# knagrecha/saturn

Hardware: AMD Instinct MI355X
Metric: samples_per_s (higher is better)
Workload: dtype bf16; 1 GPU; model=gptj-6b, global_batch=16, seq_len=512, parallelism=dp1, optimizer=fused_sgd

## Files before the change

saturn_amd/models/gptj.py:

```python

from __future__ import annotations


import os
from dataclasses import dataclass

import torch
import torch.nn as nn

from saturn_amd.ops.functional import (
    fused_gelu,
    FusedLayerNorm,
    apply_rope,
    causal_attention,
    fused_add3,
    fused_cross_entropy,
    rope_tables,
    FusedDropout,
    FusedEmbedding,
    gptj_mlp,
    mlp_fused_supported,
    gptj_branches,
    gptj_branches_supported,
)


@dataclass
class GPTJConfig:
    vocab_size: int = 50400
    n_ctx: int = 512
    n_embd: int = 4096
    n_head: int = 16
    n_layer: int = 28
    rotary_dim: int = 64
    embd_pdrop: float = 0.0
    resid_pdrop: float = 0.0


class GPTJAttention(nn.Module):
    def __init__(self, cfg: GPTJConfig):
        super().__init__()
        self.n_head = cfg.n_head
        self.head_dim = cfg.n_embd // cfg.n_head
        self.rotary_dim = cfg.rotary_dim
        E = cfg.n_embd
        self.q_proj = nn.Linear(E, E, bias=False)
        self.k_proj = nn.Linear(E, E, bias=False)
        self.v_proj = nn.Linear(E, E, bias=False)
        self.out_proj = nn.Linear(E, E, bias=False)
        self.n_ctx = cfg.n_ctx
        self._rope_f32 = rope_tables(cfg.n_ctx, cfg.rotary_dim)

    def _rope(self, device):
        if self._rope_f32[0].device != device:
            self._rope_f32 = tuple(t.to(device) for t in self._rope_f32)
        return self._rope_f32

    def forward(self, x):
        B, T, E = x.shape
        H, D = self.n_head, self.head_dim
        q = self.q_proj(x).view(B, T, H, D)
        k = self.k_proj(x).view(B, T, H, D)
        v = self.v_proj(x).view(B, T, H, D)
        cos, sin = self._rope(x.device)
        q = apply_rope(q, cos, sin)
        k = apply_rope(k, cos, sin)
        q = q.transpose(1, 2)
        k = k.transpose(1, 2)
        v = v.transpose(1, 2)
        o = causal_attention(q, k, v)
        o = o.transpose(1, 2).reshape(B, T, -1)
        return self.out_proj(o)


class GPTJMLP(nn.Module):
    def __init__(self, cfg: GPTJConfig):
        super().__init__()
        E = cfg.n_embd
        self.fc_in = nn.Linear(E, 4 * E)
        self.fc_out = nn.Linear(4 * E, E)

    @staticmethod
    def _plain_linear(m) -> bool:
        return type(m) is nn.Linear and not (
            m._forward_hooks
            or m._forward_pre_hooks
            or m._backward_hooks
            or m._backward_pre_hooks
        )

    def _use_fused(self, x) -> bool:
        if os.environ.get("SAMD_MLP_FUSED", "1") == "0":
            return False
        fi, fo = self.fc_in, self.fc_out
        return (
            x.is_cuda
            and self._plain_linear(fi)
            and self._plain_linear(fo)
            and mlp_fused_supported(x, fi.weight, fi.bias, fo.weight, fo.bias)
        )

    def forward(self, x):
        if self._use_fused(x):
            fi, fo = self.fc_in, self.fc_out
            return gptj_mlp(x, fi.weight, fi.bias, fo.weight, fo.bias)
        return self.fc_out(fused_gelu(self.fc_in(x)))


class GPTJBlock(nn.Module):

    def __init__(self, cfg: GPTJConfig):
        super().__init__()
        self.ln_1 = FusedLayerNorm(cfg.n_embd)
        self.attn = GPTJAttention(cfg)
        self.mlp = GPTJMLP(cfg)
        self.drop = FusedDropout(cfg.resid_pdrop)

    @staticmethod
    def _hooked(m) -> bool:
        return bool(
            m._forward_hooks
            or m._forward_pre_hooks
            or m._backward_hooks
            or m._backward_pre_hooks
        )

    def _use_fused(self, h) -> bool:
        if (os.environ.get("SAMD_MLP_FUSED", "1") == "0"
                or os.environ.get("SAMD_BLOCK_FUSED", "1") == "0"):
            return False
        attn, mlp = self.attn, self.mlp
        if type(attn) is not GPTJAttention or type(mlp) is not GPTJMLP:
            return False
        if not (h.is_cuda and h.dtype == torch.bfloat16 and h.dim() == 3):
            return False
        if self.drop.p != 0.0:
            return False
        from saturn_amd.parallel.sequence import sp_world

        if sp_world() != 1:
            return False
        if any(self._hooked(m) for b in (attn, mlp, self.drop) for m in b.modules()):
            return False
        projs = (attn.q_proj, attn.k_proj, attn.v_proj, attn.out_proj)
        fi, fo = mlp.fc_in, mlp.fc_out
        if not all(GPTJMLP._plain_linear(m) for m in (*projs, fi, fo)):
            return False
        E = h.shape[-1]
        if any(m.bias is not None or m.weight.shape != (E, E)
               or m.weight.dtype != torch.bfloat16 or not m.weight.is_cuda
               for m in projs):
            return False
        return mlp_fused_supported(
            h, fi.weight, fi.bias, fo.weight, fo.bias
        ) and gptj_branches_supported(
            h, attn.n_head, attn.rotary_dim, attn._rope_f32[0].shape[0]
        )

    def forward(self, x):
        h = self.ln_1(x)
        if self._use_fused(h):
            attn, mlp = self.attn, self.mlp
            cos, sin = attn._rope(h.device)
            a, m = gptj_branches(
                h, attn.q_proj.weight, attn.k_proj.weight, attn.v_proj.weight,
                attn.out_proj.weight, mlp.fc_in.weight, mlp.fc_in.bias,
                mlp.fc_out.weight, mlp.fc_out.bias, cos, sin, attn.n_head,
            )
            return fused_add3(x, a, m)
        return fused_add3(x, self.drop(self.attn(h)), self.drop(self.mlp(h)))


class GPTJForCausalLM(nn.Module):
    def __init__(self, cfg: GPTJConfig):
        super().__init__()
        self.cfg = cfg
        self.wte = FusedEmbedding(cfg.vocab_size, cfg.n_embd)
        self.drop = FusedDropout(cfg.embd_pdrop)
        self.h = nn.ModuleList(GPTJBlock(cfg) for _ in range(cfg.n_layer))
        self.ln_f = FusedLayerNorm(cfg.n_embd)
        self.lm_head = nn.Linear(cfg.n_embd, cfg.vocab_size, bias=True)
        self.apply(self._init)

    @staticmethod
    def _init(m):
        if isinstance(m, nn.Linear):
            nn.init.normal_(m.weight, std=0.02)
            if m.bias is not None:
                nn.init.zeros_(m.bias)
        elif isinstance(m, nn.Embedding):
            nn.init.normal_(m.weight, std=0.02)

    def forward(self, input_ids):
        x = self.drop(self.wte(input_ids))
        for block in self.h:
            x = block(x)
        x = self.ln_f(x)
        return self.lm_head(x)


def pretraining_loss(logits, labels):
    return fused_cross_entropy(logits, labels, shift=True)


class _EmbedStage(nn.Module):
    def __init__(self, wte):
        super().__init__()
        self.wte = wte

    def forward(self, input_ids):
        return self.wte(input_ids)


class _HeadStage(nn.Module):
    def __init__(self, ln_f, lm_head):
        super().__init__()
        self.ln_f = ln_f
        self.lm_head = lm_head

    def forward(self, x):
        return self.lm_head(self.ln_f(x))


def as_sequential(model: GPTJForCausalLM) -> nn.Sequential:
    return nn.Sequential(
        _EmbedStage(model.wte), *model.h, _HeadStage(model.ln_f, model.lm_head)
    )


def get_gptj_model(kwargs=None):
    kwargs = kwargs or {}
    cfg = GPTJConfig(
        n_layer=kwargs.get("n_layer", 28),
        n_embd=kwargs.get("n_embd", 4096),
        n_head=kwargs.get("n_head", 16),
        n_ctx=kwargs.get("n_ctx", 512),
        vocab_size=kwargs.get("vocab_size", 50400),
        rotary_dim=kwargs.get("rotary_dim", 64),
        embd_pdrop=kwargs.get("embd_pdrop", 0.0),
        resid_pdrop=kwargs.get("resid_pdrop", 0.0),
    )
    torch.manual_seed(kwargs.get("seed", 0))
    return GPTJForCausalLM(cfg)


class SyntheticTokens(torch.utils.data.Dataset):

    def __init__(self, n: int, seq_len: int, vocab: int, seed: int = 1):
        g = torch.Generator().manual_seed(seed)
        self.data = torch.randint(0, vocab, (n, seq_len), generator=g)

    def __len__(self):
        return len(self.data)

    def __getitem__(self, i):
        return self.data[i]


def _collate(batch):
    x = torch.stack(batch)
    return x, x.clone()


def make_token_dataloader(batch_size=8, seq_len=512, vocab=50400, n_batches=64):
    def get_dataloader():
        return torch.utils.data.DataLoader(
            SyntheticTokens(batch_size * n_batches, seq_len, vocab),
            batch_size=batch_size,
            shuffle=False,
            collate_fn=_collate,
        )

    return get_dataloader
```

saturn_amd/ops/csrc/attention.hip:

```cpp

#include <torch/extension.h>
#include <ATen/hip/HIPContext.h>

#include "common.h"

namespace samd {

typedef __attribute__((ext_vector_type(8))) short bf16x8;
typedef __attribute__((ext_vector_type(4))) float f32x4;

constexpr int QBLK = 64;
constexpr int KBLK = 32;
constexpr int WROWS = 16;

struct TStr {
  long sb, sh, st;
};
static TStr str_of(const at::Tensor& t) {
  return TStr{t.stride(0), t.stride(1), t.stride(2)};
}


typedef __attribute__((ext_vector_type(4))) short bf16x4;

__device__ __forceinline__ unsigned lds_addr32(const unsigned short* p) {
  return (unsigned)(unsigned long long)(
      __attribute__((address_space(3))) const unsigned short*)p;
}

template <int P1, int P2>
__device__ __forceinline__ void tr16_bfrag2(const unsigned short* t1_row0,
                                            const unsigned short* t2_row0,
                                            int lane, bf16x8& o1, bf16x8& o2) {
  const int src_row = (lane >> 2) & 3;
  const int src_col = 4 * (lane & 3);
  const unsigned a0 = lds_addr32(t1_row0 + src_row * P1 + src_col);
  const unsigned a1 = a0 + 4u * P1 * 2u;
  const unsigned b0 = lds_addr32(t2_row0 + src_row * P2 + src_col);
  const unsigned b1 = b0 + 4u * P2 * 2u;
  bf16x4 v0, v1, w0, w1;
  asm volatile(
      "ds_read_b64_tr_b16 %0, %4\n\t"
      "ds_read_b64_tr_b16 %1, %5\n\t"
      "ds_read_b64_tr_b16 %2, %6\n\t"
      "ds_read_b64_tr_b16 %3, %7\n\t"
      "s_waitcnt lgkmcnt(0)"
      : "=&v"(v0), "=&v"(v1), "=&v"(w0), "=&v"(w1)
      : "v"(a0), "v"(a1), "v"(b0), "v"(b1)
      : "memory");
  o1 = __builtin_shufflevector(v0, v1, 0, 1, 2, 3, 4, 5, 6, 7);
  o2 = __builtin_shufflevector(w0, w1, 0, 1, 2, 3, 4, 5, 6, 7);
}

template <int ROWPITCH>
__device__ __forceinline__ bf16x8 tr16_bfrag(const unsigned short* tile_row0,
                                             int lane) {
  const int src_row = (lane >> 2) & 3;
  const int src_col = 4 * (lane & 3);
  const unsigned a0 =
      lds_addr32(tile_row0 + src_row * ROWPITCH + src_col);
  const unsigned a1 = a0 + 4u * ROWPITCH * 2u;
  bf16x4 v0, v1;
  asm volatile(
      "ds_read_b64_tr_b16 %0, %2\n\t"
      "ds_read_b64_tr_b16 %1, %3\n\t"
      "s_waitcnt lgkmcnt(0)"
      : "=&v"(v0), "=&v"(v1)
      : "v"(a0), "v"(a1)
      : "memory");
  return __builtin_shufflevector(v0, v1, 0, 1, 2, 3, 4, 5, 6, 7);
}

template <int D>
struct AttnLds {
  unsigned short k[KBLK][D + 8];
  unsigned short v[KBLK][D + 8];
  unsigned short p[4][WROWS][KBLK];
};

template <int D>
__launch_bounds__(256, 2)
__global__ void attn_fwd_kernel(const unsigned short* __restrict__ Q,
                                const unsigned short* __restrict__ K,
                                const unsigned short* __restrict__ V,
                                unsigned short* __restrict__ O,
                                float* __restrict__ LSE, int T, int n_heads,
                                int n_kv, float scale, int causal,
                                int kv_len, TStr qs, TStr ks, TStr vs,
                                TStr os) {
  extern __shared__ __attribute__((aligned(16))) char smem[];
  AttnLds<D>& lds = *reinterpret_cast<AttnLds<D>*>(smem);

  const int lane = threadIdx.x & 63;
  const int wid = threadIdx.x >> 6;
  const int q0_block = blockIdx.y * QBLK;
  const int q0 = q0_block + wid * WROWS;
  const long bh = blockIdx.x;
  const long b = bh / n_heads, h = bh % n_heads;
  const long h_kv = h * n_kv / n_heads;
  const unsigned short* Qh = Q + b * qs.sb + h * qs.sh;
  const unsigned short* Kh = K + b * ks.sb + h_kv * ks.sh;
  const unsigned short* Vh = V + b * vs.sb + h_kv * vs.sh;

  const int r = lane & 15;
  const int qg = lane >> 4;

  bf16x8 frag_q[D / 32];
#pragma unroll
  for (int ds = 0; ds < D / 32; ++ds) {
    const unsigned short* src = Qh + (long)(q0 + r) * qs.st + ds * 32 + qg * 8;
    frag_q[ds] = *reinterpret_cast<const bf16x8*>(src);
  }

  f32x4 otile[D / 16];
#pragma unroll
  for (int dt = 0; dt < D / 16; ++dt) otile[dt] = {0.f, 0.f, 0.f, 0.f};

  float m_reg[4] = {-INFINITY, -INFINITY, -INFINITY, -INFINITY};
  float l_reg[4] = {0.f, 0.f, 0.f, 0.f};

  const int kv_end = causal ? (q0_block + QBLK) : T;
  constexpr int CHUNKS = (KBLK * D) / (256 * 8);
  bf16x8 stg_k[CHUNKS], stg_v[CHUNKS];
#pragma unroll
  for (int c = 0; c < CHUNKS; ++c) {
    const int idx = (c * 256 + threadIdx.x) * 8;
    const int row = idx / D, col = idx % D;
    stg_k[c] = *reinterpret_cast<const bf16x8*>(Kh + (long)row * ks.st + col);
    stg_v[c] = *reinterpret_cast<const bf16x8*>(Vh + (long)row * vs.st + col);
  }
  for (int kv0 = 0; kv0 < kv_end; kv0 += KBLK) {
    __syncthreads();
#pragma unroll
    for (int c = 0; c < CHUNKS; ++c) {
      const int idx = (c * 256 + threadIdx.x) * 8;
      const int row = idx / D, col = idx % D;
      *reinterpret_cast<bf16x8*>(&lds.k[row][col]) = stg_k[c];
      *reinterpret_cast<bf16x8*>(&lds.v[row][col]) = stg_v[c];
    }
    if (kv0 + KBLK < kv_end) {
#pragma unroll
      for (int c = 0; c < CHUNKS; ++c) {
        const int idx = (c * 256 + threadIdx.x) * 8;
        const int row = idx / D, col = idx % D;
        stg_k[c] = *reinterpret_cast<const bf16x8*>(
            Kh + (long)(kv0 + KBLK + row) * ks.st + col);
        stg_v[c] = *reinterpret_cast<const bf16x8*>(
            Vh + (long)(kv0 + KBLK + row) * vs.st + col);
      }
    }
    __syncthreads();

    f32x4 acc0 = {0.f, 0.f, 0.f, 0.f};
    f32x4 acc1 = {0.f, 0.f, 0.f, 0.f};
#pragma unroll
    for (int ds = 0; ds < D / 32; ++ds) {
      bf16x8 bk0 = *reinterpret_cast<const bf16x8*>(&lds.k[r][ds * 32 + qg * 8]);
      bf16x8 bk1 =
          *reinterpret_cast<const bf16x8*>(&lds.k[16 + r][ds * 32 + qg * 8]);
      acc0 = __builtin_amdgcn_mfma_f32_16x16x32_bf16(frag_q[ds], bk0, acc0, 0, 0, 0);
      acc1 = __builtin_amdgcn_mfma_f32_16x16x32_bf16(frag_q[ds], bk1, acc1, 0, 0, 0);
    }
#pragma unroll
    for (int reg = 0; reg < 4; ++reg) {
      const int row = qg * 4 + reg;
      const int qrow = q0 + row;
      float s0 = acc0[reg] * scale;
      float s1 = acc1[reg] * scale;
      if (causal) {
        if (kv0 + r > qrow) s0 = -INFINITY;
        if (kv0 + 16 + r > qrow) s1 = -INFINITY;
      }
      if (kv0 + r >= kv_len) s0 = -INFINITY;
      if (kv0 + 16 + r >= kv_len) s1 = -INFINITY;
      float tm = fmaxf(s0, s1);
#pragma unroll
      for (int off = 1; off < 16; off <<= 1)
        tm = fmaxf(tm, __shfl_xor(tm, off, 64));
      const float m_new = fmaxf(m_reg[reg], tm);
      const float al =
          (m_reg[reg] == -INFINITY) ? 0.f : __expf(m_reg[reg] - m_new);
      const float p0 = (s0 == -INFINITY) ? 0.f : __expf(s0 - m_new);
      const float p1 = (s1 == -INFINITY) ? 0.f : __expf(s1 - m_new);
      float ps = p0 + p1;
#pragma unroll
      for (int off = 1; off < 16; off <<= 1)
        ps += __shfl_xor(ps, off, 64);
      l_reg[reg] = l_reg[reg] * al + ps;
      m_reg[reg] = m_new;
      lds.p[wid][row][r] = f2us(p0);
      lds.p[wid][row][16 + r] = f2us(p1);
#pragma unroll
      for (int dt = 0; dt < D / 16; ++dt) otile[dt][reg] *= al;
    }

    bf16x8 frag_p = *reinterpret_cast<const bf16x8*>(&lds.p[wid][r][qg * 8]);
#pragma unroll
    for (int dt = 0; dt < D / 16; ++dt) {
      bf16x8 bv = tr16_bfrag<D + 8>(&lds.v[qg * 8][dt * 16], lane);
      otile[dt] = __builtin_amdgcn_mfma_f32_16x16x32_bf16(frag_p, bv, otile[dt], 0, 0, 0);
    }
  }

  unsigned short* Oh = O + b * os.sb + h * os.sh;
#pragma unroll
  for (int reg = 0; reg < 4; ++reg) {
    int row = qg * 4 + reg;
    float linv = 1.f / l_reg[reg];
#pragma unroll
    for (int dt = 0; dt < D / 16; ++dt)
      Oh[(long)(q0 + row) * os.st + dt * 16 + r] =
          f2us(otile[dt][reg] * linv);
  }
  if (r == 0 && LSE != nullptr) {
#pragma unroll
    for (int reg = 0; reg < 4; ++reg)
      LSE[bh * (long)T + q0 + qg * 4 + reg] =
          m_reg[reg] + __logf(l_reg[reg]);
  }
}



typedef __attribute__((ext_vector_type(16))) float f32x16;

template <int D>
struct AttnV2Lds {
  unsigned short k[KBLK][D + 8];
  unsigned short v[KBLK][D + 8];
};

template <int D>
__launch_bounds__(256, 2)
__global__ void attn_fwd_v2_kernel(const unsigned short* __restrict__ Q,
                                   const unsigned short* __restrict__ K,
                                   const unsigned short* __restrict__ V,
                                   unsigned short* __restrict__ O,
                                   float* __restrict__ LSE, int T,
                                   int n_heads, int n_kv, float scale,
                                   int causal, int kv_len, TStr qs,
                                   TStr ks, TStr vs,
                                   TStr os) {
  extern __shared__ __attribute__((aligned(16))) char smem[];
  AttnV2Lds<D>& lds = *reinterpret_cast<AttnV2Lds<D>*>(smem);

  const int lane = threadIdx.x & 63;
  const int wid = threadIdx.x >> 6;
  const int qr = lane & 31;
  const int hi = lane >> 5;
  const long bh = blockIdx.x;
  const long b = bh / n_heads, h = bh % n_heads;
  const long h_kv = h * n_kv / n_heads;
  const int q0_block = blockIdx.y * (4 * 32);
  const int q0 = q0_block + wid * 32;
  const unsigned short* Qh = Q + b * qs.sb + h * qs.sh;
  const unsigned short* Kh = K + b * ks.sb + h_kv * ks.sh;
  const unsigned short* Vh = V + b * vs.sb + h_kv * vs.sh;

  constexpr bool QREG = (D < 256);
  bf16x8 frag_q[QREG ? D / 16 : 1];
  if constexpr (QREG) {
#pragma unroll
    for (int ds = 0; ds < D / 16; ++ds)
      frag_q[ds] = *reinterpret_cast<const bf16x8*>(
          Qh + (long)(q0 + qr) * qs.st + ds * 16 + hi * 8);
  }

  f32x16 oacc[D / 32];
#pragma unroll
  for (int dv = 0; dv < D / 32; ++dv)
#pragma unroll
    for (int e = 0; e < 16; ++e) oacc[dv][e] = 0.f;

  float m_row = -INFINITY, l_row = 0.f;

  constexpr int CHUNKS = (KBLK * D) / (256 * 8);
  bf16x8 stg_k[CHUNKS], stg_v[CHUNKS];
#pragma unroll
  for (int c = 0; c < CHUNKS; ++c) {
    const int idx = (c * 256 + threadIdx.x) * 8;
    const int row = idx / D, col = idx % D;
    stg_k[c] = *reinterpret_cast<const bf16x8*>(Kh + (long)row * ks.st + col);
    stg_v[c] = *reinterpret_cast<const bf16x8*>(Vh + (long)row * vs.st + col);
  }

  const int kv_end = causal ? (q0_block + 4 * 32) : T;
  for (int kv0 = 0; kv0 < kv_end; kv0 += KBLK) {
    __syncthreads();
#pragma unroll
    for (int c = 0; c < CHUNKS; ++c) {
      const int idx = (c * 256 + threadIdx.x) * 8;
      const int row = idx / D, col = idx % D;
      *reinterpret_cast<bf16x8*>(&lds.k[row][col]) = stg_k[c];
      *reinterpret_cast<bf16x8*>(&lds.v[row][col]) = stg_v[c];
    }
    if (kv0 + KBLK < kv_end) {
#pragma unroll
      for (int c = 0; c < CHUNKS; ++c) {
        const int idx = (c * 256 + threadIdx.x) * 8;
        const int row = idx / D, col = idx % D;
        stg_k[c] = *reinterpret_cast<const bf16x8*>(
            Kh + (long)(kv0 + KBLK + row) * ks.st + col);
        stg_v[c] = *reinterpret_cast<const bf16x8*>(
            Vh + (long)(kv0 + KBLK + row) * vs.st + col);
      }
    }
    __syncthreads();

    f32x16 st;
#pragma unroll
    for (int e = 0; e < 16; ++e) st[e] = 0.f;
#pragma unroll
    for (int ds = 0; ds < D / 16; ++ds) {
      bf16x8 ak = *reinterpret_cast<const bf16x8*>(
          &lds.k[qr][ds * 16 + hi * 8]);
      bf16x8 fq;
      if constexpr (QREG)
        fq = frag_q[ds];
      else
        fq = *reinterpret_cast<const bf16x8*>(
            Qh + (long)(q0 + qr) * qs.st + ds * 16 + hi * 8);
      st = __builtin_amdgcn_mfma_f32_32x32x16_bf16(ak, fq, st, 0, 0, 0);
    }

    const int q_glob = q0 + qr;
    float p[16];
    float tile_max = -INFINITY;
#pragma unroll
    for (int reg = 0; reg < 16; ++reg) {
      const int key_loc = (reg & 3) + 8 * (reg >> 2) + 4 * hi;
      float sv = st[reg] * scale;
      if ((causal && kv0 + key_loc > q_glob) || kv0 + key_loc >= kv_len)
        sv = -INFINITY;
      p[reg] = sv;
      tile_max = fmaxf(tile_max, sv);
    }
    tile_max = fmaxf(tile_max, __shfl_xor(tile_max, 32, 64));
    const float m_new = fmaxf(m_row, tile_max);
    const float alpha = (m_row == -INFINITY) ? 0.f : __expf(m_row - m_new);
    float psum = 0.f;
#pragma unroll
    for (int reg = 0; reg < 16; ++reg) {
      const float pv = (p[reg] == -INFINITY) ? 0.f : __expf(p[reg] - m_new);
      p[reg] = pv;
      psum += pv;
    }
    psum += __shfl_xor(psum, 32, 64);
    l_row = l_row * alpha + psum;
    m_row = m_new;

    unsigned pk[8];
#pragma unroll
    for (int i = 0; i < 8; ++i) {
      const unsigned lo = f2us(p[2 * i]);
      const unsigned hi2 = f2us(p[2 * i + 1]);
      pk[i] = lo | (hi2 << 16);
    }
    bf16x8 pa[2];
#pragma unroll
    for (int g = 0; g < 2; ++g) {
      auto r0 = __builtin_amdgcn_permlane32_swap(pk[4 * g + 0], pk[4 * g + 2],
                                                 false, false);
      auto r1 = __builtin_amdgcn_permlane32_swap(pk[4 * g + 1], pk[4 * g + 3],
                                                 false, false);
      unsigned w0 = r0[0], w1 = r1[0], w2 = r0[1], w3 = r1[1];
      pa[g][0] = (short)(w0 & 0xffff);
      pa[g][1] = (short)(w0 >> 16);
      pa[g][2] = (short)(w1 & 0xffff);
      pa[g][3] = (short)(w1 >> 16);
      pa[g][4] = (short)(w2 & 0xffff);
      pa[g][5] = (short)(w2 >> 16);
      pa[g][6] = (short)(w3 & 0xffff);
      pa[g][7] = (short)(w3 >> 16);
    }

#pragma unroll
    for (int reg = 0; reg < 16; ++reg) {
      const int row = (reg & 3) + 8 * (reg >> 2) + 4 * hi;
      const float al = __shfl(alpha, row, 64);
#pragma unroll
      for (int dv = 0; dv < D / 32; ++dv) oacc[dv][reg] *= al;
    }

#pragma unroll
    for (int dv = 0; dv < D / 32; ++dv) {
#pragma unroll
      for (int g = 0; g < 2; ++g) {
        const int src_row = g * 16 + ((lane >> 4) & 2) * 4 + ((lane >> 2) & 3);
        const int src_col = dv * 32 + ((lane >> 4) & 1) * 16 + 4 * (lane & 3);
        const unsigned a0 = lds_addr32(&lds.v[src_row][src_col]);
        const unsigned a1 = a0 + 4u * (D + 8) * 2u;
        bf16x4 v0, v1;
        asm volatile(
            "ds_read_b64_tr_b16 %0, %2\n\t"
            "ds_read_b64_tr_b16 %1, %3\n\t"
            "s_waitcnt lgkmcnt(0)"
            : "=&v"(v0), "=&v"(v1)
            : "v"(a0), "v"(a1)
            : "memory");
        bf16x8 bv = __builtin_shufflevector(v0, v1, 0, 1, 2, 3, 4, 5, 6, 7);
        oacc[dv] = __builtin_amdgcn_mfma_f32_32x32x16_bf16(pa[g], bv,
                                                           oacc[dv], 0, 0, 0);
      }
    }
  }

  unsigned short* Oh = O + b * os.sb + h * os.sh;
  const float linv_own = 1.f / l_row;
#pragma unroll
  for (int reg = 0; reg < 16; ++reg) {
    const int row = (reg & 3) + 8 * (reg >> 2) + 4 * hi;
    const float linv = __shfl(linv_own, row, 64);
#pragma unroll
    for (int dv = 0; dv < D / 32; ++dv)
      Oh[(long)(q0 + row) * os.st + dv * 32 + qr] = f2us(oacc[dv][reg] * linv);
  }
  if (hi == 0 && LSE != nullptr)
    LSE[bh * (long)T + q0 + qr] = m_row + __logf(l_row);
}



static bool env_is(const char* name, char c) {
  const char* e = getenv(name);
  return e && e[0] == c;
}
static bool sw_v2() {
  static const bool v = !env_is("SAMD_ATTN_V2", '0');
  return v;
}
static bool sw_tr16() {
  static const bool v = !env_is("SAMD_ATTN_BWD_TR16", '0');
  return v;
}
static bool sw_dq_gkv() {
  static const bool v = env_is("SAMD_ATTN_DQ_GKV", '1');
  return v;
}
static bool sw_vl2() {
  static const bool v = env_is("SAMD_ATTN_BWD_VL2", '1');
  return v;
}
static bool fwd_is_v2(int T, int D) {
  return sw_v2() && T % 128 == 0 && D <= 128;
}
static bool bwd_is_tr16(int D) { return sw_tr16() && D <= 128; }
static bool bwd_is_vl2(int D) { return sw_vl2() && D <= 128; }
static bool dq_is_gkv(int D) { return sw_dq_gkv() && D > 128; }

std::string attn_dispatch(int64_t T, int64_t D) {
  TORCH_CHECK(T > 0 && T % QBLK == 0, "attn_dispatch: T must be a multiple of 64");
  TORCH_CHECK(D == 64 || D == 128 || D == 256, "attn_dispatch: D in {64,128,256}");
  const int t = (int)T, d = (int)D;
  const std::string ds = std::to_string(d);
  const bool gkv = dq_is_gkv(d);
  return std::string(fwd_is_v2(t, d) ? "attn_fwd_v2_kernel<" : "attn_fwd_kernel<") +
         ds + "> attn_delta_kernel<" + ds + "> attn_bwd_kernel<" + ds + "," +
         (bwd_is_tr16(d) ? "1," : "0,") + (bwd_is_vl2(d) ? "1>" : "0>") +
         " attn_dq_kernel<" + ds + "," +
         (!gkv && bwd_is_tr16(d) ? "1," : "0,") + (gkv ? "1>" : "0>");
}

std::vector<at::Tensor> attn_fwd(at::Tensor q, at::Tensor k, at::Tensor v,
                                 bool causal, int64_t kv_len) {
  TORCH_CHECK(q.is_cuda() && q.scalar_type() == at::kBFloat16,
              "attn_fwd: bf16 only");
  TORCH_CHECK(q.dim() == 4, "attn_fwd: [B, H, T, D]");
  TORCH_CHECK(q.stride(3) == 1 && k.stride(3) == 1 && v.stride(3) == 1,
              "attn_fwd: innermost dim must be dense");
  const int B = (int)q.size(0), H = (int)q.size(1), T = (int)q.size(2),
            D = (int)q.size(3);
  const int Hkv = (int)k.size(1);
  TORCH_CHECK(H % Hkv == 0, "attn_fwd: q heads must be a multiple of kv heads");
  TORCH_CHECK(k.size(2) == T, "attn_fwd: q/k length mismatch");
  TORCH_CHECK(T % QBLK == 0, "attn_fwd: T must be a multiple of 64");
  if (kv_len <= 0) kv_len = T;
  TORCH_CHECK(kv_len <= T, "attn_fwd: kv_len exceeds padded T");
  TORCH_CHECK(D == 64 || D == 128 || D == 256, "attn_fwd: D in {64,128,256}");
  TORCH_CHECK((reinterpret_cast<uintptr_t>(q.data_ptr()) & 15) == 0 &&
              q.stride(2) % 8 == 0 && k.stride(2) % 8 == 0 &&
              v.stride(2) % 8 == 0, "attn_fwd: rows must be 16-B aligned");

  auto o_phys = at::empty({B, T, H, D}, q.options());
  auto o = o_phys.permute({0, 2, 1, 3});
  auto lse = at::empty({B, H, T}, q.options().dtype(at::kFloat));
  auto stream = at::hip::getCurrentHIPStream();
  const float scale = 1.f / sqrtf((float)D);

  if (fwd_is_v2(T, D)) {
    dim3 grid2(B * H, T / 128), block2(256);
#define LAUNCH_V2(DD)                                                        \
    do {                                                                     \
      size_t shmem = sizeof(AttnV2Lds<DD>);                                  \
      hipLaunchKernelGGL((attn_fwd_v2_kernel<DD>), grid2, block2, shmem,     \
                         stream.stream(),                                    \
                         reinterpret_cast<const unsigned short*>(q.data_ptr()), \
                         reinterpret_cast<const unsigned short*>(k.data_ptr()), \
                         reinterpret_cast<const unsigned short*>(v.data_ptr()), \
                         reinterpret_cast<unsigned short*>(o.data_ptr()),    \
                         lse.data_ptr<float>(), T, H, Hkv, scale,            \
                         causal ? 1 : 0, (int)kv_len, str_of(q), str_of(k),  \
                         str_of(v), str_of(o));                              \
    } while (0)
    if (D == 64) LAUNCH_V2(64);
    else LAUNCH_V2(128);
#undef LAUNCH_V2
    return {o, lse};
  }
  dim3 grid(B * H, T / QBLK), block(256);

#define LAUNCH(DD)                                                          \
  do {                                                                      \
    size_t shmem = sizeof(AttnLds<DD>);                                     \
    hipLaunchKernelGGL((attn_fwd_kernel<DD>), grid, block, shmem,           \
                       stream.stream(),                                     \
                       reinterpret_cast<const unsigned short*>(q.data_ptr()), \
                       reinterpret_cast<const unsigned short*>(k.data_ptr()), \
                       reinterpret_cast<const unsigned short*>(v.data_ptr()), \
                       reinterpret_cast<unsigned short*>(o.data_ptr()),     \
                       lse.data_ptr<float>(), T, H, Hkv, scale,             \
                       causal ? 1 : 0, (int)kv_len, str_of(q), str_of(k),   \
                       str_of(v), str_of(o));                               \
  } while (0)

  if (D == 64) LAUNCH(64);
  else if (D == 128) LAUNCH(128);
  else LAUNCH(256);
#undef LAUNCH
  return {o, lse};
}

}


namespace samd {

namespace bwd {
constexpr int KB = 64;
constexpr int QT = 32;
}

template <int D, bool HASV>
struct AttnBwdLds {
  unsigned short kt[bwd::KB][D + 8];
  unsigned short vt[HASV ? bwd::KB : 1][D + 8];
  unsigned short qt[bwd::QT][D + 8];
  unsigned short dot[bwd::QT][D + 8];
  unsigned short pt[4][16][bwd::QT + 8];
  unsigned short dst[bwd::KB][bwd::QT + 8];
  float lse_t[bwd::QT];
  float delta_t[bwd::QT];
};


template <int D>
__global__ void attn_delta_kernel(const unsigned short* __restrict__ dO,
                                  const unsigned short* __restrict__ O,
                                  float* __restrict__ delta, int T,
                                  int n_heads, TStr dos, TStr os) {
  const int lane = threadIdx.x & 63;
  const int wid = threadIdx.x >> 6;
  const long bh = blockIdx.y;
  const long b = bh / n_heads, h = bh % n_heads;
  const unsigned short* dOh = dO + b * dos.sb + h * dos.sh;
  const unsigned short* Oh = O + b * os.sb + h * os.sh;
  constexpr int EPL = D / 64;
  for (int t = blockIdx.x * 4 + wid; t < T; t += gridDim.x * 4) {
    float acc = 0.f;
    if constexpr (EPL >= 4) {
#pragma unroll
      for (int c = 0; c < EPL / 4; ++c) {
        const int off = (lane * (EPL / 4) + c * 64) * 4;
        bf16x4 a = *reinterpret_cast<const bf16x4*>(dOh + (long)t * dos.st + off);
        bf16x4 o4 = *reinterpret_cast<const bf16x4*>(Oh + (long)t * os.st + off);
#pragma unroll
        for (int e = 0; e < 4; ++e)
          acc += us2f((unsigned short)a[e]) * us2f((unsigned short)o4[e]);
      }
    } else {
#pragma unroll
      for (int e = 0; e < EPL; ++e) {
        const int off = lane * EPL + e;
        acc += us2f(dOh[(long)t * dos.st + off]) *
               us2f(Oh[(long)t * os.st + off]);
      }
    }
    acc = wave_allsum(acc);
    if (lane == 0) delta[bh * (long)T + t] = acc;
  }
}

template <int D, bool TR16, bool VL2>
__launch_bounds__(256, 2)
__global__ void attn_bwd_kernel(const unsigned short* __restrict__ dO,
                                const unsigned short* __restrict__ Q,
                                const unsigned short* __restrict__ K,
                                const unsigned short* __restrict__ V,
                                const float* __restrict__ LSE,
                                const float* __restrict__ DELTA,
                                unsigned short* __restrict__ dK,
                                unsigned short* __restrict__ dV,
                                float* __restrict__ dKf,
                                float* __restrict__ dVf, int T, int n_heads,
                                int n_kv, float scale, int causal,
                                int kv_len, TStr dos,
                                TStr qs, TStr ks, TStr vs,
                                TStr dks, TStr dvs) {
  using namespace bwd;
  extern __shared__ __attribute__((aligned(16))) char smem[];
  constexpr bool HASV = (D <= 128) && !VL2;
  AttnBwdLds<D, HASV>& lds = *reinterpret_cast<AttnBwdLds<D, HASV>*>(smem);

  const int lane = threadIdx.x & 63;
  const int wid = threadIdx.x >> 6;
  const int r = lane & 15;
  const int qg = lane >> 4;
  const int kv0 = blockIdx.y * KB;
  const long bh = blockIdx.x;
  const long b = bh / n_heads, h = bh % n_heads;
  const long h_kv = h * n_kv / n_heads;
  const unsigned short* Qh = Q + b * qs.sb + h * qs.sh;
  const unsigned short* Kh = K + b * ks.sb + h_kv * ks.sh;
  const unsigned short* Vh = V + b * vs.sb + h_kv * vs.sh;
  const unsigned short* dOh = dO + b * dos.sb + h * dos.sh;
  const float* lse_h = LSE + bh * (long)T;
  const float* del_h = DELTA + bh * (long)T;

  {
    constexpr int CHUNKS = (KB * D) / (256 * 8);
#pragma unroll
    for (int c = 0; c < CHUNKS; ++c) {
      int idx = (c * 256 + threadIdx.x) * 8;
      int row = idx / D, col = idx % D;
      *reinterpret_cast<bf16x8*>(&lds.kt[row][col]) =
          *reinterpret_cast<const bf16x8*>(
              Kh + (long)(kv0 + row) * ks.st + col);
      if constexpr (HASV)
        *reinterpret_cast<bf16x8*>(&lds.vt[row][col]) =
            *reinterpret_cast<const bf16x8*>(
                Vh + (long)(kv0 + row) * vs.st + col);
    }
  }

  f32x4 acc_dv[D / 16], acc_dk[D / 16];
#pragma unroll
  for (int dt = 0; dt < D / 16; ++dt) {
    acc_dv[dt] = {0.f, 0.f, 0.f, 0.f};
    acc_dk[dt] = {0.f, 0.f, 0.f, 0.f};
  }

  const int q_start = causal ? kv0 : 0;
  for (int q0 = q_start; q0 < T; q0 += QT) {
    __syncthreads();
    {
      constexpr int CHUNKS = (QT * D) / (256 * 8);
#pragma unroll
      for (int c = 0; c < CHUNKS; ++c) {
        int idx = (c * 256 + threadIdx.x) * 8;
        int row = idx / D, col = idx % D;
        *reinterpret_cast<bf16x8*>(&lds.qt[row][col]) =
            *reinterpret_cast<const bf16x8*>(
                Qh + (long)(q0 + row) * qs.st + col);
        *reinterpret_cast<bf16x8*>(&lds.dot[row][col]) =
            *reinterpret_cast<const bf16x8*>(
                dOh + (long)(q0 + row) * dos.st + col);
      }
      if (threadIdx.x < QT) {
        lds.lse_t[threadIdx.x] = lse_h[q0 + threadIdx.x];
        lds.delta_t[threadIdx.x] = del_h[q0 + threadIdx.x];
      }
    }
    __syncthreads();

#pragma unroll
    for (int n = 0; n < 2; ++n) {
      f32x4 st = {0.f, 0.f, 0.f, 0.f};
      f32x4 dpt = {0.f, 0.f, 0.f, 0.f};
#pragma unroll
      for (int ds = 0; ds < D / 32; ++ds) {
        bf16x8 ak = *reinterpret_cast<const bf16x8*>(
            &lds.kt[wid * 16 + r][ds * 32 + qg * 8]);
        bf16x8 av;
        if constexpr (HASV)
          av = *reinterpret_cast<const bf16x8*>(
              &lds.vt[wid * 16 + r][ds * 32 + qg * 8]);
        else
          av = *reinterpret_cast<const bf16x8*>(
              Vh + (long)(kv0 + wid * 16 + r) * vs.st + ds * 32 + qg * 8);
        bf16x8 bq = *reinterpret_cast<const bf16x8*>(
            &lds.qt[n * 16 + r][ds * 32 + qg * 8]);
        bf16x8 bdo = *reinterpret_cast<const bf16x8*>(
            &lds.dot[n * 16 + r][ds * 32 + qg * 8]);
        st = __builtin_amdgcn_mfma_f32_16x16x32_bf16(ak, bq, st, 0, 0, 0);
        dpt = __builtin_amdgcn_mfma_f32_16x16x32_bf16(av, bdo, dpt, 0, 0, 0);
      }
#pragma unroll
      for (int reg = 0; reg < 4; ++reg) {
        const int key_loc = qg * 4 + reg;
        const int key_glob = kv0 + wid * 16 + key_loc;
        const int q_glob = q0 + n * 16 + r;
        float p = 0.f;
        if ((!causal || q_glob >= key_glob) && key_glob < kv_len) {
          p = __expf(scale * st[reg] - lds.lse_t[n * 16 + r]);
        }
        const float dsv = p * (dpt[reg] - lds.delta_t[n * 16 + r]) * scale;
        lds.pt[wid][key_loc][n * 16 + r] = f2us(p);
        lds.dst[wid * 16 + key_loc][n * 16 + r] = f2us(dsv);
      }
    }

    {
      bf16x8 ap = *reinterpret_cast<const bf16x8*>(&lds.pt[wid][r][qg * 8]);
      bf16x8 adst =
          *reinterpret_cast<const bf16x8*>(&lds.dst[wid * 16 + r][qg * 8]);
#pragma unroll
      for (int dt = 0; dt < D / 16; ++dt) {
        bf16x8 bdo, bq;
        if constexpr (TR16) {
          tr16_bfrag2<D + 8, D + 8>(&lds.dot[qg * 8][dt * 16],
                                    &lds.qt[qg * 8][dt * 16], lane, bdo, bq);
        } else {
#pragma unroll
          for (int j = 0; j < 8; ++j) {
            bdo[j] = (short)lds.dot[qg * 8 + j][dt * 16 + r];
            bq[j] = (short)lds.qt[qg * 8 + j][dt * 16 + r];
          }
        }
        acc_dv[dt] =
            __builtin_amdgcn_mfma_f32_16x16x32_bf16(ap, bdo, acc_dv[dt], 0, 0, 0);
        acc_dk[dt] =
            __builtin_amdgcn_mfma_f32_16x16x32_bf16(adst, bq, acc_dk[dt], 0, 0, 0);
      }
    }

    __syncthreads();
  }

  if (n_kv != n_heads) {
    float* dKh = dKf + b * dks.sb + h_kv * dks.sh;
    float* dVh = dVf + b * dvs.sb + h_kv * dvs.sh;
#pragma unroll
    for (int reg = 0; reg < 4; ++reg) {
      const int key_glob = kv0 + wid * 16 + qg * 4 + reg;
#pragma unroll
      for (int dt = 0; dt < D / 16; ++dt) {
        atomicAdd(&dKh[(long)key_glob * dks.st + dt * 16 + r],
                  acc_dk[dt][reg]);
        atomicAdd(&dVh[(long)key_glob * dvs.st + dt * 16 + r],
                  acc_dv[dt][reg]);
      }
    }
  } else {
    unsigned short* dKh = dK + b * dks.sb + h * dks.sh;
    unsigned short* dVh = dV + b * dvs.sb + h * dvs.sh;
#pragma unroll
    for (int reg = 0; reg < 4; ++reg) {
      const int key_glob = kv0 + wid * 16 + qg * 4 + reg;
#pragma unroll
      for (int dt = 0; dt < D / 16; ++dt) {
        dKh[(long)key_glob * dks.st + dt * 16 + r] = f2us(acc_dk[dt][reg]);
        dVh[(long)key_glob * dvs.st + dt * 16 + r] = f2us(acc_dv[dt][reg]);
      }
    }
  }
}

namespace dq {
constexpr int QB = 64;
constexpr int KT = 32;
}

template <int D, bool GKV>
struct AttnDqLds {
  unsigned short qt[GKV ? 1 : dq::QB][D + 8];
  unsigned short dot[GKV ? 1 : dq::QB][D + 8];
  unsigned short kt[dq::KT][D + 8];
  unsigned short vt[GKV ? 1 : dq::KT][D + 8];
  float lse_t[dq::QB];
  float delta_t[dq::QB];
};

template <int D, bool TR16, bool GKV>
__launch_bounds__(256, GKV ? 3 : (D <= 128 ? 2 : 1))
__global__ void attn_dq_kernel(const unsigned short* __restrict__ dO,
                               const unsigned short* __restrict__ Q,
                               const unsigned short* __restrict__ K,
                               const unsigned short* __restrict__ V,
                               const float* __restrict__ LSE,
                               const float* __restrict__ DELTA,
                               unsigned short* __restrict__ dQ16, int T,
                               int n_heads, int n_kv, float scale, int causal,
                               int kv_len, TStr dos, TStr qs, TStr ks,
                               TStr vs, TStr dqs) {
  using namespace dq;
  extern __shared__ __attribute__((aligned(16))) char smem[];
  AttnDqLds<D, GKV>& lds = *reinterpret_cast<AttnDqLds<D, GKV>*>(smem);

  const int lane = threadIdx.x & 63;
  const int wid = threadIdx.x >> 6;
  const int r = lane & 15;
  const int qg = lane >> 4;
  const int q0 = blockIdx.y * QB;
  const long bh = blockIdx.x;
  const long b = bh / n_heads, h = bh % n_heads;
  const long h_kv = h * n_kv / n_heads;
  const unsigned short* Qh = Q + b * qs.sb + h * qs.sh;
  const unsigned short* Kh = K + b * ks.sb + h_kv * ks.sh;
  const unsigned short* Vh = V + b * vs.sb + h_kv * vs.sh;
  const unsigned short* dOh = dO + b * dos.sb + h * dos.sh;
  const float* lse_h = LSE + bh * (long)T;
  const float* del_h = DELTA + bh * (long)T;

  {
    if constexpr (!GKV) {
      constexpr int CHUNKS = (QB * D) / (256 * 8);
#pragma unroll
      for (int c = 0; c < CHUNKS; ++c) {
        int idx = (c * 256 + threadIdx.x) * 8;
        int row = idx / D, col = idx % D;
        *reinterpret_cast<bf16x8*>(&lds.qt[row][col]) =
            *reinterpret_cast<const bf16x8*>(Qh + (long)(q0 + row) * qs.st + col);
        *reinterpret_cast<bf16x8*>(&lds.dot[row][col]) =
            *reinterpret_cast<const bf16x8*>(
                dOh + (long)(q0 + row) * dos.st + col);
      }
    }
    if (threadIdx.x < QB) {
      lds.lse_t[threadIdx.x] = lse_h[q0 + threadIdx.x];
      lds.delta_t[threadIdx.x] = del_h[q0 + threadIdx.x];
    }
  }

  f32x4 acc[D / 16];
#pragma unroll
  for (int dt = 0; dt < D / 16; ++dt) acc[dt] = {0.f, 0.f, 0.f, 0.f};

  const int k_end = causal ? (q0 + QB < T ? q0 + QB : T) : T;
  for (int k0 = 0; k0 < k_end; k0 += KT) {
    __syncthreads();
    {
      constexpr int CHUNKS = (KT * D) / (256 * 8);
#pragma unroll
      for (int c = 0; c < CHUNKS; ++c) {
        int idx = (c * 256 + threadIdx.x) * 8;
        int row = idx / D, col = idx % D;
        *reinterpret_cast<bf16x8*>(&lds.kt[row][col]) =
            *reinterpret_cast<const bf16x8*>(
                Kh + (long)(k0 + row) * ks.st + col);
        if constexpr (!GKV)
          *reinterpret_cast<bf16x8*>(&lds.vt[row][col]) =
              *reinterpret_cast<const bf16x8*>(
                  Vh + (long)(k0 + row) * vs.st + col);
      }
    }
    __syncthreads();

    if (causal && k0 > q0 + wid * 16 + 15) continue;

    float ds_sub[2][4];
#pragma unroll
    for (int n = 0; n < 2; ++n) {
      f32x4 st = {0.f, 0.f, 0.f, 0.f};
      f32x4 dpt = {0.f, 0.f, 0.f, 0.f};
#pragma unroll
      for (int ds_ = 0; ds_ < D / 32; ++ds_) {
        bf16x8 ak = *reinterpret_cast<const bf16x8*>(
            &lds.kt[n * 16 + r][ds_ * 32 + qg * 8]);
        bf16x8 av, bq, bdo;
        if constexpr (GKV) {
          av = *reinterpret_cast<const bf16x8*>(
              Vh + (long)(k0 + n * 16 + r) * vs.st + ds_ * 32 + qg * 8);
          bq = *reinterpret_cast<const bf16x8*>(
              Qh + (long)(q0 + wid * 16 + r) * qs.st + ds_ * 32 + qg * 8);
          bdo = *reinterpret_cast<const bf16x8*>(
              dOh + (long)(q0 + wid * 16 + r) * dos.st + ds_ * 32 + qg * 8);
        } else {
          av = *reinterpret_cast<const bf16x8*>(
              &lds.vt[n * 16 + r][ds_ * 32 + qg * 8]);
          bq = *reinterpret_cast<const bf16x8*>(
              &lds.qt[wid * 16 + r][ds_ * 32 + qg * 8]);
          bdo = *reinterpret_cast<const bf16x8*>(
              &lds.dot[wid * 16 + r][ds_ * 32 + qg * 8]);
        }
        st = __builtin_amdgcn_mfma_f32_16x16x32_bf16(ak, bq, st, 0, 0, 0);
        dpt = __builtin_amdgcn_mfma_f32_16x16x32_bf16(av, bdo, dpt, 0, 0, 0);
      }
      const int q_glob = q0 + wid * 16 + r;
      const float l_q = lds.lse_t[wid * 16 + r];
      const float d_q = lds.delta_t[wid * 16 + r];
#pragma unroll
      for (int reg = 0; reg < 4; ++reg) {
        const int key_glob = k0 + n * 16 + qg * 4 + reg;
        float p = 0.f;
        if ((!causal || q_glob >= key_glob) && key_glob < kv_len)
          p = __expf(scale * st[reg] - l_q);
        ds_sub[n][reg] = p * (dpt[reg] - d_q) * scale;
      }
    }

    unsigned pk[2][2];
#pragma unroll
    for (int n = 0; n < 2; ++n) {
      pk[n][0] = (unsigned)f2us(ds_sub[n][0]) |
                 ((unsigned)f2us(ds_sub[n][1]) << 16);
      pk[n][1] = (unsigned)f2us(ds_sub[n][2]) |
                 ((unsigned)f2us(ds_sub[n][3]) << 16);
    }
    const int a = (qg & 1) * 2;
    const int nsrc = qg >> 1;
    const int s0 = a * 16 + r;
    const int s1 = (a + 1) * 16 + r;
    unsigned rr[4][2];
#pragma unroll
    for (int nn = 0; nn < 2; ++nn) {
      rr[nn * 2 + 0][0] = (unsigned)__shfl((int)pk[nn][0], s0, 64);
      rr[nn * 2 + 0][1] = (unsigned)__shfl((int)pk[nn][1], s0, 64);
      rr[nn * 2 + 1][0] = (unsigned)__shfl((int)pk[nn][0], s1, 64);
      rr[nn * 2 + 1][1] = (unsigned)__shfl((int)pk[nn][1], s1, 64);
    }
    bf16x8 ads;
#pragma unroll
    for (int j = 0; j < 8; ++j) {
      const int src = (j >= 4) ? 1 : 0;
      const int reg = j & 3;
      const unsigned u = rr[nsrc * 2 + src][reg >> 1];
      ads[j] = (short)((reg & 1) ? (u >> 16) : (u & 0xffffu));
    }

#pragma unroll
    for (int dt = 0; dt < D / 16; ++dt) {
      bf16x8 bk;
      if constexpr (TR16) {
        bk = tr16_bfrag<D + 8>(&lds.kt[qg * 8][dt * 16], lane);
      } else {
#pragma unroll
        for (int j = 0; j < 8; ++j)
          bk[j] = (short)lds.kt[qg * 8 + j][dt * 16 + r];
      }
      acc[dt] = __builtin_amdgcn_mfma_f32_16x16x32_bf16(ads, bk, acc[dt], 0, 0, 0);
    }
  }

  unsigned short* dQh = dQ16 + b * dqs.sb + h * dqs.sh;
#pragma unroll
  for (int reg = 0; reg < 4; ++reg) {
    const int q_glob = q0 + wid * 16 + qg * 4 + reg;
#pragma unroll
    for (int dt = 0; dt < D / 16; ++dt)
      dQh[(long)q_glob * dqs.st + dt * 16 + r] = f2us(acc[dt][reg]);
  }
}

std::vector<at::Tensor> attn_bwd(at::Tensor dout, at::Tensor q, at::Tensor k,
                                 at::Tensor v, at::Tensor o, at::Tensor lse,
                                 bool causal, int64_t kv_len) {
  using namespace bwd;
  TORCH_CHECK(q.is_cuda() && q.scalar_type() == at::kBFloat16);
  const int B = (int)q.size(0), H = (int)q.size(1), T = (int)q.size(2),
            D = (int)q.size(3);
  const int Hkv = (int)k.size(1);
  TORCH_CHECK(H % Hkv == 0);
  TORCH_CHECK(T % KB == 0, "attn_bwd: T must be a multiple of 64");
  if (kv_len <= 0) kv_len = T;
  TORCH_CHECK(kv_len <= T, "attn_bwd: kv_len exceeds padded T");
  TORCH_CHECK(D == 64 || D == 128 || D == 256);
  TORCH_CHECK(dout.stride(3) == 1 && q.stride(3) == 1 && k.stride(3) == 1 &&
              v.stride(3) == 1, "attn_bwd: innermost dim must be dense");
  TORCH_CHECK(dout.stride(2) % 8 == 0 && q.stride(2) % 8 == 0 &&
              k.stride(2) % 8 == 0 && v.stride(2) % 8 == 0);

  auto delta = at::empty({B, H, T}, q.options().dtype(at::kFloat));
  auto dq = at::empty({B, T, H, D}, q.options()).permute({0, 2, 1, 3});
  const bool gqa = Hkv != H;
  auto dk = at::empty({B, T, Hkv, D}, k.options()).permute({0, 2, 1, 3});
  auto dv = at::empty({B, T, Hkv, D}, v.options()).permute({0, 2, 1, 3});
  at::Tensor dk_f32, dv_f32;
  if (gqa) {
    dk_f32 = at::zeros({B, T, Hkv, D}, q.options().dtype(at::kFloat))
                 .permute({0, 2, 1, 3});
    dv_f32 = at::zeros({B, T, Hkv, D}, q.options().dtype(at::kFloat))
                 .permute({0, 2, 1, 3});
  }
  auto stream = at::hip::getCurrentHIPStream();
  const float scale = 1.f / sqrtf((float)D);
  dim3 grid(B * H, T / KB), block(256);

#define BWD_ARGS                                                             \
    stream.stream(),                                                         \
    reinterpret_cast<const unsigned short*>(dout.data_ptr()),                \
    reinterpret_cast<const unsigned short*>(q.data_ptr()),                   \
    reinterpret_cast<const unsigned short*>(k.data_ptr()),                   \
    reinterpret_cast<const unsigned short*>(v.data_ptr()),                   \
    lse.data_ptr<float>(), delta.data_ptr<float>(),                          \
    reinterpret_cast<unsigned short*>(dk.data_ptr()),                        \
    reinterpret_cast<unsigned short*>(dv.data_ptr()),                        \
    gqa ? dk_f32.data_ptr<float>() : nullptr,                                \
    gqa ? dv_f32.data_ptr<float>() : nullptr, T, H, Hkv,                     \
    scale, causal ? 1 : 0, (int)kv_len, str_of(dout), str_of(q),             \
    str_of(k), str_of(v),                                                    \
    gqa ? str_of(dk_f32) : str_of(dk),                                       \
    gqa ? str_of(dv_f32) : str_of(dv)

#define LAUNCH_B(DD)                                                         \
  do {                                                                       \
    dim3 dgrid(std::min((T + 3) / 4, 2048), B * H), dblock(256);             \
    hipLaunchKernelGGL((attn_delta_kernel<DD>), dgrid, dblock, 0,            \
                       stream.stream(),                                      \
                       reinterpret_cast<const unsigned short*>(dout.data_ptr()), \
                       reinterpret_cast<const unsigned short*>(o.data_ptr()), \
                       delta.data_ptr<float>(), T, H, str_of(dout),          \
                       str_of(o));                                           \
                                                           \
    const bool gkv = dq_is_gkv(DD);                                          \
    size_t SH_DQ = gkv ? sizeof(AttnDqLds<DD, true>)                         \
                       : sizeof(AttnDqLds<DD, false>);                       \
    static bool dq_attr_##DD = [] {                                          \
      hipFuncSetAttribute(                                                   \
          reinterpret_cast<const void*>(&attn_dq_kernel<DD, false, false>),  \
          hipFuncAttributeMaxDynamicSharedMemorySize,                        \
          (int)sizeof(AttnDqLds<DD, false>));                                \
      hipFuncSetAttribute(                                                   \
          reinterpret_cast<const void*>(&attn_dq_kernel<DD, true, false>),   \
          hipFuncAttributeMaxDynamicSharedMemorySize,                        \
          (int)sizeof(AttnDqLds<DD, false>));                                \
      return true;                                                           \
    }();                                                                     \
    (void)dq_attr_##DD;                                                      \
    {                                                                        \
      dim3 qgrid(B * H, T / dq::QB), qblock(256);                            \
      if (gkv)                                                               \
        hipLaunchKernelGGL((attn_dq_kernel<DD, false, true>), qgrid,         \
                           qblock, SH_DQ, stream.stream(),                   \
                           reinterpret_cast<const unsigned short*>(dout.data_ptr()), \
                           reinterpret_cast<const unsigned short*>(q.data_ptr()), \
                           reinterpret_cast<const unsigned short*>(k.data_ptr()), \
                           reinterpret_cast<const unsigned short*>(v.data_ptr()), \
                           lse.data_ptr<float>(), delta.data_ptr<float>(),   \
                           reinterpret_cast<unsigned short*>(dq.data_ptr()), \
                           T, H, Hkv, scale, causal ? 1 : 0, (int)kv_len,   \
                           str_of(dout), str_of(q), str_of(k), str_of(v),    \
                           str_of(dq));                                      \
      else if (bwd_is_tr16(DD))                                              \
        hipLaunchKernelGGL((attn_dq_kernel<DD, true, false>), qgrid,         \
                           qblock, SH_DQ, stream.stream(),                   \
                           reinterpret_cast<const unsigned short*>(dout.data_ptr()), \
                           reinterpret_cast<const unsigned short*>(q.data_ptr()), \
                           reinterpret_cast<const unsigned short*>(k.data_ptr()), \
                           reinterpret_cast<const unsigned short*>(v.data_ptr()), \
                           lse.data_ptr<float>(), delta.data_ptr<float>(),   \
                           reinterpret_cast<unsigned short*>(dq.data_ptr()), \
                           T, H, Hkv, scale, causal ? 1 : 0, (int)kv_len,   \
                           str_of(dout), str_of(q), str_of(k), str_of(v),    \
                           str_of(dq));                                      \
      else                                                                   \
        hipLaunchKernelGGL((attn_dq_kernel<DD, false, false>), qgrid,        \
                           qblock, SH_DQ, stream.stream(),                   \
                           reinterpret_cast<const unsigned short*>(dout.data_ptr()), \
                           reinterpret_cast<const unsigned short*>(q.data_ptr()), \
                           reinterpret_cast<const unsigned short*>(k.data_ptr()), \
                           reinterpret_cast<const unsigned short*>(v.data_ptr()), \
                           lse.data_ptr<float>(), delta.data_ptr<float>(),   \
                           reinterpret_cast<unsigned short*>(dq.data_ptr()), \
                           T, H, Hkv, scale, causal ? 1 : 0, (int)kv_len,   \
                           str_of(dout), str_of(q), str_of(k), str_of(v),    \
                           str_of(dq));                                      \
    }                                                                        \
    const bool tr = bwd_is_tr16(DD);                                         \
    const bool vl2 = bwd_is_vl2(DD);                                         \
    constexpr size_t SH_V = sizeof(AttnBwdLds<DD, (DD <= 128)>);             \
    constexpr size_t SH_N = sizeof(AttnBwdLds<DD, false>);                   \
    size_t shmem = vl2 ? SH_N : SH_V;                                        \
    static bool attr_set_##DD = [] {                                         \
      hipFuncSetAttribute(                                                   \
          reinterpret_cast<const void*>(&attn_bwd_kernel<DD, false, false>), \
          hipFuncAttributeMaxDynamicSharedMemorySize, (int)SH_V);            \
      hipFuncSetAttribute(                                                   \
          reinterpret_cast<const void*>(&attn_bwd_kernel<DD, true, false>),  \
          hipFuncAttributeMaxDynamicSharedMemorySize, (int)SH_V);            \
      hipFuncSetAttribute(                                                   \
          reinterpret_cast<const void*>(&attn_bwd_kernel<DD, false, true>),  \
          hipFuncAttributeMaxDynamicSharedMemorySize, (int)SH_N);            \
      hipFuncSetAttribute(                                                   \
          reinterpret_cast<const void*>(&attn_bwd_kernel<DD, true, true>),   \
          hipFuncAttributeMaxDynamicSharedMemorySize, (int)SH_N);            \
      return true;                                                           \
    }();                                                                     \
    (void)attr_set_##DD;                                                     \
    if (tr && vl2)                                                           \
      hipLaunchKernelGGL((attn_bwd_kernel<DD, true, true>), grid, block,     \
                         shmem, BWD_ARGS);                                   \
    else if (tr)                                                             \
      hipLaunchKernelGGL((attn_bwd_kernel<DD, true, false>), grid, block,    \
                         shmem, BWD_ARGS);                                   \
    else if (vl2)                                                            \
      hipLaunchKernelGGL((attn_bwd_kernel<DD, false, true>), grid, block,    \
                         shmem, BWD_ARGS);                                   \
    else                                                                     \
      hipLaunchKernelGGL((attn_bwd_kernel<DD, false, false>), grid, block,   \
                         shmem, BWD_ARGS);                                   \
  } while (0)

  if (D == 64) LAUNCH_B(64);
  else if (D == 128) LAUNCH_B(128);
  else LAUNCH_B(256);
#undef LAUNCH_B
  if (gqa) return {dq, dk_f32.to(at::kBFloat16), dv_f32.to(at::kBFloat16)};
  return {dq, dk, dv};
}

}
```

saturn_amd/ops/csrc/bindings.cpp:

```cpp

#include <torch/extension.h>
#include <vector>

namespace samd {
void fused_sgd(std::vector<at::Tensor> params, std::vector<at::Tensor> grads,
               std::vector<at::Tensor> moms, std::vector<at::Tensor> masters,
               double lr, double momentum, double weight_decay);
void fused_adam(std::vector<at::Tensor> params, std::vector<at::Tensor> grads,
                std::vector<at::Tensor> ms, std::vector<at::Tensor> vs,
                std::vector<at::Tensor> masters, double lr, double beta1,
                double beta2, double eps, double weight_decay, double bc1,
                double bc2);
std::vector<at::Tensor> norm_fwd(at::Tensor x, at::Tensor w,
                                 c10::optional<at::Tensor> b, double eps,
                                 bool rms);
std::vector<at::Tensor> norm_bwd(at::Tensor dy, at::Tensor x, at::Tensor w,
                                 at::Tensor mean, at::Tensor rstd, bool rms,
                                 bool needs_db);
std::vector<at::Tensor> ce_fwd(at::Tensor logits, at::Tensor targets,
                               int64_t Tr, int64_t ignore_index);
at::Tensor ce_bwd(at::Tensor logits, at::Tensor targets, at::Tensor lse,
                  at::Tensor dloss, int64_t Tr, int64_t ignore_index);
void rope_apply(at::Tensor y, at::Tensor x, at::Tensor cos_t, at::Tensor sin_t,
                int64_t t_len, int64_t t_off, bool half_style, bool backward);
at::Tensor gelu_fwd(at::Tensor x);
at::Tensor gelu_bwd(at::Tensor dy, at::Tensor x);
std::vector<at::Tensor> attn_fwd(at::Tensor q, at::Tensor k, at::Tensor v,
                                 bool causal, int64_t kv_len);
std::vector<at::Tensor> attn_bwd(at::Tensor dout, at::Tensor q, at::Tensor k,
                                 at::Tensor v, at::Tensor o, at::Tensor lse,
                                 bool causal, int64_t kv_len);
std::string attn_dispatch(int64_t T, int64_t D);
at::Tensor add3(at::Tensor a, at::Tensor b, at::Tensor c);
at::Tensor swiglu_fwd(at::Tensor gate, at::Tensor up);
std::vector<at::Tensor> swiglu_bwd(at::Tensor dout, at::Tensor gate,
                                   at::Tensor up);
at::Tensor embed_fwd(at::Tensor weight, at::Tensor idx);
at::Tensor embed_bwd(at::Tensor dout, at::Tensor idx, long vocab);
at::Tensor dropout_fwd(at::Tensor x, double p, long seed);
at::Tensor dropout_bwd(at::Tensor dout, double p, long seed);
std::vector<at::Tensor> moe_route_fwd(at::Tensor logits, int64_t top_k,
                                      at::ScalarType out_dtype);
at::Tensor moe_route_bwd(at::Tensor logits, at::Tensor ids,
                         at::Tensor dweights);
std::vector<at::Tensor> moe_sort(at::Tensor ids, int64_t n_expert);
at::Tensor moe_permute_fwd(at::Tensor x, at::Tensor order, int64_t top_k);
at::Tensor moe_permute_bwd(at::Tensor dxs, at::Tensor pos);
at::Tensor moe_combine_fwd(at::Tensor y, at::Tensor weights, at::Tensor pos);
std::vector<at::Tensor> moe_combine_bwd(at::Tensor dout, at::Tensor y,
                                        at::Tensor weights, at::Tensor pos);
std::vector<at::Tensor> mlp_act_bwd(at::Tensor d_act, at::Tensor pre,
                                    bool want_dT, bool want_aT);
std::vector<at::Tensor> transpose_colsum(at::Tensor x, bool want_sum);
std::vector<at::Tensor> mlp_bwd(at::Tensor g, at::Tensor h, at::Tensor pre,
                                at::Tensor W_in, at::Tensor W_out,
                                bool use_tn_in, bool use_tn_out);
void transpose_into(at::Tensor x, at::Tensor dst);
at::Tensor rope_bwd_t(at::Tensor dy, at::Tensor cos_t, at::Tensor sin_t,
                      int64_t t_len, int64_t t_off, int64_t dim,
                      at::Tensor dxT);
std::vector<at::Tensor> gptj_branches_bwd(
    at::Tensor g_a, at::Tensor g_m, at::Tensor h, at::Tensor pre, at::Tensor q,
    at::Tensor k, at::Tensor v, at::Tensor o, at::Tensor lse, at::Tensor Wq,
    at::Tensor Wk, at::Tensor Wv, at::Tensor Wo, at::Tensor W_in,
    at::Tensor W_out, at::Tensor cos_t, at::Tensor sin_t, int64_t t_off,
    bool tn_in, bool tn_out, bool tn_qkv, bool tn_o, bool dh_accum);
}

PYBIND11_MODULE(TORCH_EXTENSION_NAME, m) {
  m.doc() = "saturn_amd hand-written CDNA4 (gfx950) kernels";
  m.def("fused_sgd", &samd::fused_sgd, "fused multi-tensor SGD");
  m.def("fused_adam", &samd::fused_adam, "fused multi-tensor AdamW");
  m.def("norm_fwd", &samd::norm_fwd, "LayerNorm/RMSNorm forward");
  m.def("norm_bwd", &samd::norm_bwd, "LayerNorm/RMSNorm backward");
  m.def("ce_fwd", &samd::ce_fwd, "fused cross-entropy forward");
  m.def("ce_bwd", &samd::ce_bwd, "fused cross-entropy backward");
  m.def("rope_apply", &samd::rope_apply,
        "fused rotary embedding (out-of-place, offset table rows)");
  m.def("gelu_fwd", &samd::gelu_fwd, "fused tanh-approx GELU forward");
  m.def("gelu_bwd", &samd::gelu_bwd, "fused tanh-approx GELU backward");
  m.def("attn_fwd", &samd::attn_fwd, "fused flash attention forward",
        py::arg("q"), py::arg("k"), py::arg("v"), py::arg("causal"),
        py::arg("kv_len") = -1);
  m.def("attn_dispatch", &samd::attn_dispatch,
        "kernel instantiations attn_fwd/attn_bwd launch for (padded T, D)",
        py::arg("T"), py::arg("D"));
  m.def("attn_bwd", &samd::attn_bwd, "fused flash attention backward",
        py::arg("dout"), py::arg("q"), py::arg("k"), py::arg("v"),
        py::arg("o"), py::arg("lse"), py::arg("causal"),
        py::arg("kv_len") = -1);
  m.def("add3", &samd::add3, "fused 3-way residual add");
  m.def("swiglu_fwd", &samd::swiglu_fwd, "fused silu(gate)*up");
  m.def("swiglu_bwd", &samd::swiglu_bwd, "fused SwiGLU backward");
  m.def("embed_fwd", &samd::embed_fwd, "token embedding gather");
  m.def("embed_bwd", &samd::embed_bwd, "embedding scatter-add backward");
  m.def("dropout_fwd", &samd::dropout_fwd, "counter-based fused dropout");
  m.def("dropout_bwd", &samd::dropout_bwd, "dropout backward (mask recompute)");
  m.def("moe_route_fwd", &samd::moe_route_fwd,
        "MoE softmax + top-k + renormalise (ties to the lower expert)");
  m.def("moe_route_bwd", &samd::moe_route_bwd, "MoE routing backward");
  m.def("moe_sort", &samd::moe_sort,
        "stable counting sort of (token, slot) pairs by expert");
  m.def("moe_permute_fwd", &samd::moe_permute_fwd,
        "gather token rows into expert order");
  m.def("moe_permute_bwd", &samd::moe_permute_bwd,
        "sum each token's k permuted rows");
  m.def("moe_combine_fwd", &samd::moe_combine_fwd,
        "weighted sum of each token's k expert rows");
  m.def("moe_combine_bwd", &samd::moe_combine_bwd,
        "combine backward: dy and fp32 dweights");
  m.def("mlp_act_bwd", &samd::mlp_act_bwd,
        "GELU backward + transposed d_pre / gelu(pre) + fp32 bias grad",
        py::arg("d_act"), py::arg("pre"), py::arg("want_dT") = true,
        py::arg("want_aT") = true);
  m.def("transpose_colsum", &samd::transpose_colsum,
        "bf16 transpose with optional fp32 column sums");
  m.def("mlp_bwd", &samd::mlp_bwd,
        "GPT-J MLP backward with TN-layout weight gradients");
  m.def("transpose_into", &samd::transpose_into,
        "bf16 transpose stored into a caller-given [N, M] view",
        py::arg("x"), py::arg("dst"));
  m.def("rope_bwd_t", &samd::rope_bwd_t,
        "interleaved RoPE backward that also stores dx^T into a [E, M] view",
        py::arg("dy"), py::arg("cos"), py::arg("sin"), py::arg("t_len"),
        py::arg("t_off"), py::arg("dim"), py::arg("dxT"));
  m.def("gptj_branches_bwd", &samd::gptj_branches_bwd,
        "GPT-J attention + MLP branch backward with shared transposes");
}
```

saturn_amd/ops/csrc/common.h:

```cpp
#pragma once

#include <hip/hip_runtime.h>
#include <hip/hip_bf16.h>
#include <hip/hip_fp16.h>

#define WAVE 64

namespace samd {

typedef __attribute__((ext_vector_type(4))) short short4v;
typedef __attribute__((ext_vector_type(8))) short short8v;
typedef __attribute__((ext_vector_type(4))) float float4v;

__device__ __forceinline__ float bf2f(__hip_bfloat16 x) {
  return __bfloat162float(x);
}
__device__ __forceinline__ __hip_bfloat16 f2bf(float x) {
  return __float2bfloat16(x);
}

template <typename T>
__device__ __forceinline__ float toF(T v) { return (float)v; }
template <>
__device__ __forceinline__ float toF<__half>(__half v) { return __half2float(v); }
template <>
__device__ __forceinline__ float toF<__hip_bfloat16>(__hip_bfloat16 v) {
  return __bfloat162float(v);
}
template <typename T>
__device__ __forceinline__ T fromF(float v) { return (T)v; }
template <>
__device__ __forceinline__ __half fromF<__half>(float v) {
  return __float2half(v);
}
template <>
__device__ __forceinline__ __hip_bfloat16 fromF<__hip_bfloat16>(float v) {
  return __float2bfloat16(v);
}

__device__ __forceinline__ float us2f(unsigned short u) {
  union { unsigned int i; float f; } c;
  c.i = ((unsigned int)u) << 16;
  return c.f;
}
__device__ __forceinline__ unsigned short f2us(float f) {
  union { unsigned int i; float f; } c;
  c.f = f;
  unsigned int lsb = (c.i >> 16) & 1u;
  unsigned int rounded = c.i + 0x7fffu + lsb;
  return (unsigned short)(rounded >> 16);
}

__device__ __forceinline__ float wave_sum(float v) {
#pragma unroll
  for (int off = 32; off > 0; off >>= 1) v += __shfl_down(v, off, 64);
  return v;
}
__device__ __forceinline__ float wave_max(float v) {
#pragma unroll
  for (int off = 32; off > 0; off >>= 1) v = fmaxf(v, __shfl_down(v, off, 64));
  return v;
}
__device__ __forceinline__ float wave_allsum(float v) {
#pragma unroll
  for (int off = 32; off > 0; off >>= 1) v += __shfl_xor(v, off, 64);
  return v;
}
__device__ __forceinline__ float wave_allmax(float v) {
#pragma unroll
  for (int off = 32; off > 0; off >>= 1) v = fmaxf(v, __shfl_xor(v, off, 64));
  return v;
}

template <int BLOCK>
__device__ __forceinline__ float block_sum(float v, float* lds ) {
  const int lane = threadIdx.x & (WAVE - 1);
  const int wid = threadIdx.x / WAVE;
  v = wave_sum(v);
  if (lane == 0) lds[wid] = v;
  __syncthreads();
  float r = 0.f;
  if (wid == 0) {
    r = (lane < BLOCK / WAVE) ? lds[lane] : 0.f;
    r = wave_sum(r);
    if (lane == 0) lds[0] = r;
  }
  __syncthreads();
  r = lds[0];
  __syncthreads();
  return r;
}

template <int BLOCK>
__device__ __forceinline__ float block_max(float v, float* lds) {
  const int lane = threadIdx.x & (WAVE - 1);
  const int wid = threadIdx.x / WAVE;
  v = wave_max(v);
  if (lane == 0) lds[wid] = v;
  __syncthreads();
  float r = -INFINITY;
  if (wid == 0) {
    r = (lane < BLOCK / WAVE) ? lds[lane] : -INFINITY;
    r = wave_max(r);
    if (lane == 0) lds[0] = r;
  }
  __syncthreads();
  r = lds[0];
  __syncthreads();
  return r;
}

}

#define SAMD_CHECK_HIP(expr)                                        \
  do {                                                              \
    hipError_t _e = (expr);                                         \
    if (_e != hipSuccess) {                                         \
      TORCH_CHECK(false, "HIP error: ", hipGetErrorString(_e));     \
    }                                                               \
  } while (0)
```

saturn_amd/ops/csrc/gptj_block_bwd.hip:

```cpp

#include <torch/extension.h>
#include <ATen/hip/HIPContext.h>

#include "common.h"
#include "tile_image.h"

namespace samd {

std::vector<at::Tensor> attn_bwd(at::Tensor dout, at::Tensor q, at::Tensor k,
                                 at::Tensor v, at::Tensor o, at::Tensor lse,
                                 bool causal, int64_t kv_len);
std::vector<at::Tensor> mlp_act_bwd(at::Tensor d_act, at::Tensor pre,
                                    bool want_dT, bool want_aT);
void rope_apply(at::Tensor y, at::Tensor x, at::Tensor cos_t, at::Tensor sin_t,
                int64_t t_len, int64_t t_off, bool half_style, bool backward);

namespace {

__global__ void __launch_bounds__(MB_BLOCK)
rope_bwd_t_kernel(const bf16_t* __restrict__ dy, bf16_t* __restrict__ dx,
                  bf16_t* __restrict__ dxT, const float* __restrict__ cos_t,
                  const float* __restrict__ sin_t, long M, long E, int t_len,
                  long t_off, int dim, int half, float sign) {
  __shared__ uint4 img[MB_TILE * 8];

  const int tid = threadIdx.x;
  const int cv = tid & 7;
  const int rp = tid >> 3;
  const int mv = tid & 7;
  const int cr = tid >> 3;
  const long col0 = (long)blockIdx.x * MB_TILE;
  const long col = col0 + cv * 8;
  const bool col_ok = col < E;
  const int j0 = (int)(col % dim);
  const bool rotary = j0 < 2 * half;

  for (int it = 0; it < MB_ROW_ITERS; ++it) {
    const long row0 = ((long)blockIdx.y * MB_ROW_ITERS + it) * MB_TILE;
    if (row0 >= M) break;
    const long row = row0 + 2 * rp;
    const bool ok = col_ok && row < M;

    const short8v zero8 = {0, 0, 0, 0, 0, 0, 0, 0};
    short8v ov[2];
#pragma unroll
    for (int i = 0; i < 2; ++i) {
      ov[i] = zero8;
      if (!ok) continue;
      const short8v xv =
          *reinterpret_cast<const short8v*>(dy + (row + i) * E + col);
      if (rotary) {
        const long trow = (t_off + ((row + i) % t_len)) * (long)half;
#pragma unroll
        for (int e = 0; e < 4; ++e) {
          const int p = j0 / 2 + e;
          const float c = cos_t[trow + p];
          const float s = sin_t[trow + p] * sign;
          bf16_t e0, e1;
          e0.x = (unsigned short)xv[2 * e];
          e1.x = (unsigned short)xv[2 * e + 1];
          const float x0 = toF<bf16_t>(e0);
          const float x1 = toF<bf16_t>(e1);
          ov[i][2 * e] = (short)fromF<bf16_t>(x0 * c - x1 * s).x;
          ov[i][2 * e + 1] = (short)fromF<bf16_t>(x1 * c + x0 * s).x;
        }
      } else {
        ov[i] = xv;
      }
      *reinterpret_cast<short8v*>(dx + (row + i) * E + col) = ov[i];
    }
    unsigned* i32 = reinterpret_cast<unsigned*>(img);
#pragma unroll
    for (int e = 0; e < 8; ++e) {
      i32[img_dword(cv * 8 + e, rp)] =
          (unsigned)(unsigned short)ov[0][e] |
          ((unsigned)(unsigned short)ov[1][e] << 16);
    }
    __syncthreads();

    const long mrow = row0 + mv * 8;
#pragma unroll
    for (int j = 0; j < 2; ++j) {
      const int c = cr + 32 * j;
      if ((col0 + c < E) && (mrow < M))
        *reinterpret_cast<uint4*>(dxT + (col0 + c) * M + mrow) =
            img[img_slot(c, mv)];
    }
    __syncthreads();
  }
}

void check_f32_table(const at::Tensor& t, const char* name) {
  TORCH_CHECK(t.is_cuda() && t.scalar_type() == at::kFloat && t.dim() == 2 &&
                  t.is_contiguous(),
              name, ": expected a contiguous fp32 [T, half] GPU tensor");
}

}

at::Tensor rope_bwd_t(at::Tensor dy, at::Tensor cos_t, at::Tensor sin_t,
                      int64_t t_len, int64_t t_off, int64_t dim,
                      at::Tensor dxT) {
  TORCH_CHECK(dy.is_cuda() && dy.scalar_type() == at::kBFloat16 &&
                  dy.is_contiguous() && dy.numel() > 0,
              "rope_bwd_t dy: expected a contiguous bf16 GPU tensor");
  check_f32_table(cos_t, "rope_bwd_t cos");
  check_f32_table(sin_t, "rope_bwd_t sin");
  const long half = cos_t.size(1);
  TORCH_CHECK(sin_t.sizes() == cos_t.sizes(), "rope_bwd_t: table mismatch");
  TORCH_CHECK(dim > 0 && dim % 8 == 0, "rope_bwd_t: head dim ", dim,
              " must be a positive multiple of 8");
  TORCH_CHECK((2 * half) % 8 == 0 && 2 * half <= dim,
              "rope_bwd_t: rotary dim ", 2 * half,
              " must be a multiple of 8 within the head dim");
  TORCH_CHECK(dy.numel() % dim == 0 && dy.size(-1) == dim,
              "rope_bwd_t: last dim of dy must be the head dim");
  TORCH_CHECK(dy.dim() >= 2, "rope_bwd_t dy: expected [..., heads, dim]");
  const long E = dy.size(-2) * dim;
  const long M = dy.numel() / E;
  TORCH_CHECK(M % 8 == 0, "rope_bwd_t: token count ", M,
              " must be a multiple of 8");
  TORCH_CHECK(t_len > 0 && M % t_len == 0,
              "rope_bwd_t: token count not a multiple of T");
  TORCH_CHECK(t_off >= 0 && cos_t.size(0) >= t_off + t_len,
              "rope_bwd_t: table too short for offset+T");
  TORCH_CHECK(reinterpret_cast<uintptr_t>(dy.data_ptr()) % 16 == 0,
              "rope_bwd_t dy: data must be 16-byte aligned");
  check_operand(dxT, "rope_bwd_t dxT");
  TORCH_CHECK(dxT.size(0) == E && dxT.size(1) == M &&
                  dxT.device() == dy.device(),
              "rope_bwd_t: dxT must be [", E, ", ", M, "], got ", dxT.sizes());

  auto dx = at::empty_like(dy);
  const dim3 grid = tile_grid(M, E);
  auto stream = at::hip::getCurrentHIPStream();
  hipLaunchKernelGGL(rope_bwd_t_kernel, grid, dim3(MB_BLOCK), 0,
                     stream.stream(), bptr(dy), bptr(dx), bptr(dxT),
                     cos_t.data_ptr<float>(), sin_t.data_ptr<float>(), M, E,
                     (int)t_len, (long)t_off, (int)dim, (int)half, -1.f);
  SAMD_CHECK_HIP(hipGetLastError());
  return dx;
}

std::vector<at::Tensor> gptj_branches_bwd(
    at::Tensor g_a, at::Tensor g_m, at::Tensor h, at::Tensor pre, at::Tensor q,
    at::Tensor k, at::Tensor v, at::Tensor o, at::Tensor lse, at::Tensor Wq,
    at::Tensor Wk, at::Tensor Wv, at::Tensor Wo, at::Tensor W_in,
    at::Tensor W_out, at::Tensor cos_t, at::Tensor sin_t, int64_t t_off,
    bool tn_in, bool tn_out, bool tn_qkv, bool tn_o, bool dh_accum) {
  check_operand(g_a, "gptj_branches_bwd g_a");
  check_operand(g_m, "gptj_branches_bwd g_m");
  check_operand(h, "gptj_branches_bwd h");
  check_operand(pre, "gptj_branches_bwd pre");
  check_operand(W_in, "gptj_branches_bwd W_in");
  check_operand(W_out, "gptj_branches_bwd W_out");
  const long M = h.size(0), E = h.size(1), F = pre.size(1);
  TORCH_CHECK(q.dim() == 4 && o.dim() == 4, "gptj_branches_bwd: q, o 4-D");
  const long B = q.size(0), H = q.size(1), T = q.size(2), D = q.size(3);
  TORCH_CHECK(B * T == M && H * D == E && k.sizes() == q.sizes() &&
                  v.sizes() == q.sizes() && o.sizes() == q.sizes(),
              "gptj_branches_bwd: attention shapes do not match h");
  TORCH_CHECK(g_a.sizes() == h.sizes() && g_m.sizes() == h.sizes() &&
                  pre.size(0) == M && W_in.size(0) == F && W_in.size(1) == E &&
                  W_out.size(0) == E && W_out.size(1) == F,
              "gptj_branches_bwd: inconsistent shapes");
  for (const at::Tensor* w : {&Wq, &Wk, &Wv, &Wo}) {
    check_operand(*w, "gptj_branches_bwd projection weight");
    TORCH_CHECK(w->size(0) == E && w->size(1) == E,
                "gptj_branches_bwd: projection weights must be [E, E]");
  }
  auto o_phys = o.permute({0, 2, 1, 3});
  TORCH_CHECK(o_phys.is_contiguous(),
              "gptj_branches_bwd: o must be physically [B,T,H,D]");
  auto o2 = o_phys.view({M, E});
  const bool shared = g_a.data_ptr() == g_m.data_ptr();

  auto gt = transpose_colsum_impl(g_m, true, tn_out || (shared && tn_o));
  at::Tensor gaT;
  if (tn_o) gaT = shared ? gt[0] : transpose_colsum_impl(g_a, false, true)[0];
  at::Tensor hT;
  if (tn_in || tn_qkv) hT = transpose_colsum_impl(h, false, true)[0];

  at::Tensor dh, dW_in, db_in, dW_out;
  {
    at::Tensor d_pre, d_preT, act;
    {
      auto d_act = at::mm(g_m, W_out);
      auto r = mlp_act_bwd(d_act, pre, tn_in, tn_out);
      d_pre = r[0];
      d_preT = r[1];
      act = r[2];
      db_in = r[3];
    }
    dW_out = tn_out ? at::linear(gt[0], act) : at::mm(g_m.t(), act);
    act.reset();
    if (!tn_o) gt[0].reset();
    dW_in = tn_in ? at::linear(d_preT, hT) : at::mm(d_pre.t(), h);
    d_preT.reset();
    if (!tn_qkv) hT.reset();
    dh = at::mm(d_pre, W_in);
  }

  auto d_o = at::mm(g_a, Wo);
  at::Tensor dWo;
  if (tn_o) {
    auto oT = transpose_colsum_impl(o2, false, true)[0];
    dWo = at::linear(gaT, oT);
    gaT.reset();
    gt[0].reset();
  } else {
    dWo = at::mm(g_a.t(), o2);
  }

  at::Tensor dq_r, dk_r, dv;
  {
    auto r = attn_bwd(d_o.view({B, T, H, D}).permute({0, 2, 1, 3}), q, k, v, o,
                      lse, true, T);
    dq_r = r[0].permute({0, 2, 1, 3});
    dk_r = r[1].permute({0, 2, 1, 3});
    dv = r[2].permute({0, 2, 1, 3});
    TORCH_CHECK(dq_r.is_contiguous() && dk_r.is_contiguous() &&
                    dv.is_contiguous(),
                "gptj_branches_bwd: attn_bwd layout changed");
  }
  d_o.reset();
  auto dv2 = dv.view({M, E});

  at::Tensor dq, dk, dWq, dWk, dWv;
  if (tn_qkv) {
    auto dqkvT = at::empty({3 * E, M}, h.options());
    dq = rope_bwd_t(dq_r, cos_t, sin_t, T, t_off, D, dqkvT.narrow(0, 0, E));
    dq_r.reset();
    dk = rope_bwd_t(dk_r, cos_t, sin_t, T, t_off, D, dqkvT.narrow(0, E, E));
    dk_r.reset();
    transpose_colsum_impl(dv2, false, true, dqkvT.narrow(0, 2 * E, E));
    auto dW = at::linear(dqkvT, hT);
    dqkvT.reset();
    hT.reset();
    dWq = dW.narrow(0, 0, E);
    dWk = dW.narrow(0, E, E);
    dWv = dW.narrow(0, 2 * E, E);
  } else {
    dq = at::empty_like(dq_r);
    rope_apply(dq, dq_r, cos_t, sin_t, T, t_off, false, true);
    dq_r.reset();
    dk = at::empty_like(dk_r);
    rope_apply(dk, dk_r, cos_t, sin_t, T, t_off, false, true);
    dk_r.reset();
    dWq = at::mm(dq.view({M, E}).t(), h);
    dWk = at::mm(dk.view({M, E}).t(), h);
    dWv = at::mm(dv2.t(), h);
  }

  auto dq2 = dq.view({M, E}), dk2 = dk.view({M, E});
  if (dh_accum) {
    dh.addmm_(dv2, Wv);
    dh.addmm_(dk2, Wk);
    dh.addmm_(dq2, Wq);
  } else {
    dh.add_(at::mm(dv2, Wv));
    dh.add_(at::mm(dk2, Wk));
    dh.add_(at::mm(dq2, Wq));
  }
  return {dh, dWq, dWk, dWv, dWo, dW_in, db_in.to(W_in.scalar_type()),
          dW_out, gt[1].to(W_out.scalar_type())};
}

}
```

saturn_amd/ops/csrc/layernorm.hip:

```cpp

#include <torch/extension.h>
#include <ATen/hip/HIPContext.h>

#include "common.h"

namespace samd {

constexpr int LN_BLOCK = 256;

typedef __attribute__((ext_vector_type(8))) short short8v_ln;

template <typename T>
__device__ __forceinline__ float elemF(const short8v_ln& v, int e) {
  T t;
  t.x = (unsigned short)v[e];
  return toF<T>(t);
}

template <typename T>
__device__ __forceinline__ void setElem(short8v_ln& v, int e, float f) {
  v[e] = (short)fromF<T>(f).x;
}


template <typename T, bool RMS, int GMAX>
__global__ void norm_fwd_vec_kernel(const T* __restrict__ x,
                                    const T* __restrict__ w,
                                    const T* __restrict__ b, T* __restrict__ y,
                                    float* __restrict__ mean_out,
                                    float* __restrict__ rstd_out, int rows,
                                    int cols, float eps) {
  __shared__ float lds[LN_BLOCK / WAVE];
  float cache[8 * GMAX];
  for (int row = blockIdx.x; row < rows; row += gridDim.x) {
    const T* xr = x + (long)row * cols;
    T* yr = y + (long)row * cols;
    float s = 0.f, sq = 0.f;
#pragma unroll
    for (int g = 0; g < GMAX; ++g) {
      const int j = (g * LN_BLOCK + threadIdx.x) * 8;
      if (j < cols) {
        const short8v_ln xv = *reinterpret_cast<const short8v_ln*>(xr + j);
#pragma unroll
        for (int e = 0; e < 8; ++e) {
          const float v = elemF<T>(xv, e);
          cache[g * 8 + e] = v;
          s += v;
          sq += v * v;
        }
      }
    }
    float mean = 0.f;
    if (!RMS) mean = block_sum<LN_BLOCK>(s, lds) / cols;
    const float var = block_sum<LN_BLOCK>(sq, lds) / cols - mean * mean;
    const float rstd = rsqrtf(var + eps);
    if (threadIdx.x == 0) {
      if (!RMS && mean_out) mean_out[row] = mean;
      if (rstd_out) rstd_out[row] = rstd;
    }
#pragma unroll
    for (int g = 0; g < GMAX; ++g) {
      const int j = (g * LN_BLOCK + threadIdx.x) * 8;
      if (j < cols) {
        const short8v_ln wv = *reinterpret_cast<const short8v_ln*>(w + j);
        short8v_ln bv;
        if (!RMS && b) bv = *reinterpret_cast<const short8v_ln*>(b + j);
        short8v_ln ov;
#pragma unroll
        for (int e = 0; e < 8; ++e) {
          const float v = (cache[g * 8 + e] - mean) * rstd;
          float o = v * elemF<T>(wv, e);
          if (!RMS && b) o += elemF<T>(bv, e);
          setElem<T>(ov, e, o);
        }
        *reinterpret_cast<short8v_ln*>(yr + j) = ov;
      }
    }
    __syncthreads();
  }
}

template <typename T, bool RMS>
__global__ void norm_fwd_kernel(const T* __restrict__ x, const T* __restrict__ w,
                                const T* __restrict__ b, T* __restrict__ y,
                                float* __restrict__ mean_out,
                                float* __restrict__ rstd_out, int rows,
                                int cols, float eps) {
  __shared__ float lds[LN_BLOCK / WAVE];
  for (int row = blockIdx.x; row < rows; row += gridDim.x) {
    const T* xr = x + (long)row * cols;
    T* yr = y + (long)row * cols;
    float s = 0.f, sq = 0.f;
    for (int j = threadIdx.x; j < cols; j += LN_BLOCK) {
      float v = (float)xr[j];
      s += v;
      sq += v * v;
    }
    float mean = 0.f;
    if (!RMS) {
      mean = block_sum<LN_BLOCK>(s, lds) / cols;
    }
    float var = block_sum<LN_BLOCK>(sq, lds) / cols - mean * mean;
    float rstd = rsqrtf(var + eps);
    if (threadIdx.x == 0) {
      if (!RMS && mean_out) mean_out[row] = mean;
      if (rstd_out) rstd_out[row] = rstd;
    }
    for (int j = threadIdx.x; j < cols; j += LN_BLOCK) {
      float v = ((float)xr[j] - mean) * rstd;
      float wv = (float)w[j];
      float o = RMS ? v * wv : v * wv + (b ? (float)b[j] : 0.f);
      yr[j] = (T)o;
    }
    __syncthreads();
  }
}


template <typename T, bool RMS, int GMAX>
__global__ void norm_bwd_vec_kernel(const T* __restrict__ dy,
                                    const T* __restrict__ x,
                                    const T* __restrict__ w,
                                    const float* __restrict__ mean,
                                    const float* __restrict__ rstd,
                                    T* __restrict__ dx, float* __restrict__ dw,
                                    float* __restrict__ db, int rows,
                                    int cols) {
  __shared__ float lds[LN_BLOCK / WAVE];
  float dwp[8 * GMAX];
  float dbp[8 * GMAX];
#pragma unroll
  for (int k = 0; k < 8 * GMAX; ++k) { dwp[k] = 0.f; dbp[k] = 0.f; }
  constexpr bool CACHE = GMAX <= 2;
  float c_dyw[CACHE ? 8 * GMAX : 1];
  float c_xh[CACHE ? 8 * GMAX : 1];
  for (int row = blockIdx.x; row < rows; row += gridDim.x) {
    const T* dyr = dy + (long)row * cols;
    const T* xr = x + (long)row * cols;
    T* dxr = dx + (long)row * cols;
    const float mu = RMS ? 0.f : mean[row];
    const float rs = rstd[row];
    float s1 = 0.f, s2 = 0.f;
#pragma unroll
    for (int g = 0; g < GMAX; ++g) {
      const int j = (g * LN_BLOCK + threadIdx.x) * 8;
      if (j < cols) {
        const short8v_ln dyv = *reinterpret_cast<const short8v_ln*>(dyr + j);
        const short8v_ln xv = *reinterpret_cast<const short8v_ln*>(xr + j);
        const short8v_ln wv = *reinterpret_cast<const short8v_ln*>(w + j);
#pragma unroll
        for (int e = 0; e < 8; ++e) {
          const float dyf = elemF<T>(dyv, e);
          const float xh = (elemF<T>(xv, e) - mu) * rs;
          const float dyw = dyf * elemF<T>(wv, e);
          if constexpr (CACHE) {
            c_dyw[g * 8 + e] = dyw;
            c_xh[g * 8 + e] = xh;
          }
          s1 += dyw;
          s2 += dyw * xh;
          dwp[g * 8 + e] += dyf * xh;
          dbp[g * 8 + e] += dyf;
        }
      }
    }
    const float m1 = RMS ? 0.f : block_sum<LN_BLOCK>(s1, lds) / cols;
    const float m2 = block_sum<LN_BLOCK>(s2, lds) / cols;
#pragma unroll
    for (int g = 0; g < GMAX; ++g) {
      const int j = (g * LN_BLOCK + threadIdx.x) * 8;
      if (j < cols) {
        short8v_ln ov;
        if constexpr (CACHE) {
#pragma unroll
          for (int e = 0; e < 8; ++e)
            setElem<T>(ov, e,
                       rs * (c_dyw[g * 8 + e] - m1 - c_xh[g * 8 + e] * m2));
        } else {
          const short8v_ln dyv = *reinterpret_cast<const short8v_ln*>(dyr + j);
          const short8v_ln xv = *reinterpret_cast<const short8v_ln*>(xr + j);
          const short8v_ln wv = *reinterpret_cast<const short8v_ln*>(w + j);
#pragma unroll
          for (int e = 0; e < 8; ++e) {
            const float dyw = elemF<T>(dyv, e) * elemF<T>(wv, e);
            const float xh = (elemF<T>(xv, e) - mu) * rs;
            setElem<T>(ov, e, rs * (dyw - m1 - xh * m2));
          }
        }
        *reinterpret_cast<short8v_ln*>(dxr + j) = ov;
      }
    }
    __syncthreads();
  }
  float* dwr = dw + (long)blockIdx.x * cols;
  float* dbr = db ? db + (long)blockIdx.x * cols : nullptr;
#pragma unroll
  for (int g = 0; g < GMAX; ++g) {
    const int j = (g * LN_BLOCK + threadIdx.x) * 8;
    if (j < cols) {
#pragma unroll
      for (int e = 0; e < 8; ++e) {
        dwr[j + e] = dwp[g * 8 + e];
        if (db) dbr[j + e] = dbp[g * 8 + e];
      }
    }
  }
}


template <typename T, bool RMS, int CPT>
__global__ void norm_bwd_kernel(const T* __restrict__ dy, const T* __restrict__ x,
                                const T* __restrict__ w,
                                const float* __restrict__ mean,
                                const float* __restrict__ rstd,
                                T* __restrict__ dx, float* __restrict__ dw,
                                float* __restrict__ db, int rows, int cols) {
  __shared__ float lds[LN_BLOCK / WAVE];
  float dwp[CPT];
  float dbp[CPT];
#pragma unroll
  for (int k = 0; k < CPT; ++k) { dwp[k] = 0.f; dbp[k] = 0.f; }

  constexpr bool CACHE = (CPT <= 16);
  float c_dyw[CACHE ? CPT : 1];
  float c_xh[CACHE ? CPT : 1];
  for (int row = blockIdx.x; row < rows; row += gridDim.x) {
    const T* dyr = dy + (long)row * cols;
    const T* xr = x + (long)row * cols;
    T* dxr = dx + (long)row * cols;
    const float mu = RMS ? 0.f : mean[row];
    const float rs = rstd[row];
    float s1 = 0.f, s2 = 0.f;
    for (int k = 0, j = threadIdx.x; j < cols; j += LN_BLOCK, ++k) {
      float dyv = (float)dyr[j];
      float xh = ((float)xr[j] - mu) * rs;
      float dyw = dyv * (float)w[j];
      if constexpr (CACHE) {
        c_dyw[k] = dyw;
        c_xh[k] = xh;
      }
      s1 += dyw;
      s2 += dyw * xh;
      dwp[k] += dyv * xh;
      dbp[k] += dyv;
    }
    float m1 = RMS ? 0.f : block_sum<LN_BLOCK>(s1, lds) / cols;
    float m2 = block_sum<LN_BLOCK>(s2, lds) / cols;
    if constexpr (CACHE) {
      for (int k = 0, j = threadIdx.x; j < cols; j += LN_BLOCK, ++k)
        dxr[j] = (T)(rs * (c_dyw[k] - m1 - c_xh[k] * m2));
    } else {
      for (int j = threadIdx.x; j < cols; j += LN_BLOCK) {
        float dyw = (float)dyr[j] * (float)w[j];
        float xh = ((float)xr[j] - mu) * rs;
        dxr[j] = (T)(rs * (dyw - m1 - xh * m2));
      }
    }
    __syncthreads();
  }
  for (int k = 0, j = threadIdx.x; j < cols; j += LN_BLOCK, ++k) {
    atomicAdd(&dw[j], dwp[k]);
    if (db) atomicAdd(&db[j], dbp[k]);
  }
}

static int norm_grid(int rows) { return std::min(rows, 2048); }

std::vector<at::Tensor> norm_fwd(at::Tensor x, at::Tensor w,
                                 c10::optional<at::Tensor> b, double eps,
                                 bool rms) {
  TORCH_CHECK(x.is_cuda() && x.is_contiguous());
  const int cols = (int)x.size(-1);
  const int rows = (int)(x.numel() / cols);
  TORCH_CHECK(cols <= 64 * LN_BLOCK, "row too long for norm kernels");
  auto y = at::empty_like(x);
  auto opts = x.options().dtype(at::kFloat);
  auto mean = rms ? at::Tensor() : at::empty({rows}, opts);
  auto rstd = at::empty({rows}, opts);
  auto stream = at::hip::getCurrentHIPStream();
  dim3 grid(norm_grid(rows)), block(LN_BLOCK);
  const bool vec_ok = x.scalar_type() != at::kFloat && cols % 8 == 0 &&
                      cols <= 8 * LN_BLOCK * 8;

  AT_DISPATCH_FLOATING_TYPES_AND2(
      at::kBFloat16, at::kHalf, x.scalar_type(), "norm_fwd", [&] {
        using T = scalar_t;
        if constexpr (sizeof(T) == 2) {
          if (vec_ok) {
            const int gneeded = (cols + 8 * LN_BLOCK - 1) / (8 * LN_BLOCK);
            void (*kv)(const T*, const T*, const T*, T*, float*, float*, int,
                       int, float);
            if (gneeded <= 2)
              kv = rms ? norm_fwd_vec_kernel<T, true, 2>
                       : norm_fwd_vec_kernel<T, false, 2>;
            else
              kv = rms ? norm_fwd_vec_kernel<T, true, 8>
                       : norm_fwd_vec_kernel<T, false, 8>;
            hipLaunchKernelGGL(kv, grid, block, 0, stream.stream(),
                               reinterpret_cast<const T*>(x.data_ptr()),
                               reinterpret_cast<const T*>(w.data_ptr()),
                               b.has_value()
                                   ? reinterpret_cast<const T*>(b->data_ptr())
                                   : nullptr,
                               reinterpret_cast<T*>(y.data_ptr()),
                               rms ? nullptr : mean.data_ptr<float>(),
                               rstd.data_ptr<float>(), rows, cols,
                               (float)eps);
            return;
          }
        }
        auto k = rms ? norm_fwd_kernel<T, true> : norm_fwd_kernel<T, false>;
        hipLaunchKernelGGL(k, grid, block, 0, stream.stream(),
                           reinterpret_cast<const T*>(x.data_ptr()),
                           reinterpret_cast<const T*>(w.data_ptr()),
                           b.has_value()
                               ? reinterpret_cast<const T*>(b->data_ptr())
                               : nullptr,
                           reinterpret_cast<T*>(y.data_ptr()),
                           rms ? nullptr : mean.data_ptr<float>(),
                           rstd.data_ptr<float>(), rows, cols, (float)eps);
      });
  return {y, mean, rstd};
}

std::vector<at::Tensor> norm_bwd(at::Tensor dy, at::Tensor x, at::Tensor w,
                                 at::Tensor mean, at::Tensor rstd, bool rms,
                                 bool needs_db) {
  TORCH_CHECK(dy.is_cuda() && dy.is_contiguous() && x.is_contiguous());
  const int cols = (int)x.size(-1);
  const int rows = (int)(x.numel() / cols);
  auto dx = at::empty_like(x);
  auto opts = x.options().dtype(at::kFloat);
  auto dw = at::zeros({cols}, opts);
  auto db = needs_db ? at::zeros({cols}, opts) : at::Tensor();
  auto stream = at::hip::getCurrentHIPStream();
  dim3 grid(norm_grid(rows)), block(LN_BLOCK);

  const int cpt_needed = (cols + LN_BLOCK - 1) / LN_BLOCK;
  const bool vec_ok =
      x.scalar_type() != at::kFloat && cols % 8 == 0 && cols <= 8 * LN_BLOCK * 4;
  AT_DISPATCH_FLOATING_TYPES_AND2(
      at::kBFloat16, at::kHalf, x.scalar_type(), "norm_bwd", [&] {
        using T = scalar_t;
        if constexpr (sizeof(T) == 2) {
          if (vec_ok) {
            const int gneeded = (cols + 8 * LN_BLOCK - 1) / (8 * LN_BLOCK);
            void (*kv)(const T*, const T*, const T*, const float*,
                       const float*, T*, float*, float*, int, int);
            if (gneeded <= 2)
              kv = rms ? norm_bwd_vec_kernel<T, true, 2>
                       : norm_bwd_vec_kernel<T, false, 2>;
            else
              kv = rms ? norm_bwd_vec_kernel<T, true, 4>
                       : norm_bwd_vec_kernel<T, false, 4>;
            const int nblk = grid.x;
            auto dw_part = at::empty({nblk, cols}, opts);
            auto db_part =
                needs_db ? at::empty({nblk, cols}, opts) : at::Tensor();
            hipLaunchKernelGGL(kv, grid, block, 0, stream.stream(),
                               reinterpret_cast<const T*>(dy.data_ptr()),
                               reinterpret_cast<const T*>(x.data_ptr()),
                               reinterpret_cast<const T*>(w.data_ptr()),
                               rms ? nullptr : mean.data_ptr<float>(),
                               rstd.data_ptr<float>(),
                               reinterpret_cast<T*>(dx.data_ptr()),
                               dw_part.data_ptr<float>(),
                               needs_db ? db_part.data_ptr<float>() : nullptr,
                               rows, cols);
            at::sum_out(dw, dw_part, {0});
            if (needs_db) at::sum_out(db, db_part, {0});
            return;
          }
        }
        void (*k)(const T*, const T*, const T*, const float*, const float*,
                  T*, float*, float*, int, int);
        if (cpt_needed <= 8)
          k = rms ? norm_bwd_kernel<T, true, 8> : norm_bwd_kernel<T, false, 8>;
        else if (cpt_needed <= 16)
          k = rms ? norm_bwd_kernel<T, true, 16> : norm_bwd_kernel<T, false, 16>;
        else if (cpt_needed <= 32)
          k = rms ? norm_bwd_kernel<T, true, 32> : norm_bwd_kernel<T, false, 32>;
        else
          k = rms ? norm_bwd_kernel<T, true, 64> : norm_bwd_kernel<T, false, 64>;
        hipLaunchKernelGGL(k, grid, block, 0, stream.stream(),
                           reinterpret_cast<const T*>(dy.data_ptr()),
                           reinterpret_cast<const T*>(x.data_ptr()),
                           reinterpret_cast<const T*>(w.data_ptr()),
                           rms ? nullptr : mean.data_ptr<float>(),
                           rstd.data_ptr<float>(),
                           reinterpret_cast<T*>(dx.data_ptr()),
                           dw.data_ptr<float>(),
                           needs_db ? db.data_ptr<float>() : nullptr, rows,
                           cols);
      });
  return {dx, dw, db};
}

}
```

saturn_amd/ops/functional.py:

```python

from __future__ import annotations

import os
from typing import Tuple

import torch
import torch.nn.functional as F

from saturn_amd.ops import require_ext


class _NormFn(torch.autograd.Function):
    @staticmethod
    def forward(ctx, x, w, b, eps, rms):
        ext = require_ext()
        x = x.contiguous()
        y, mean, rstd = ext.norm_fwd(x, w, b, eps, rms)
        if rms:
            mean = rstd
        ctx.save_for_backward(x, w, mean, rstd)
        ctx.rms = rms
        ctx.has_b = b is not None
        return y

    @staticmethod
    def backward(ctx, dy):
        ext = require_ext()
        x, w, mean, rstd = ctx.saved_tensors
        dx, dw, db = ext.norm_bwd(
            dy.contiguous(), x, w, mean, rstd, ctx.rms, ctx.has_b
        )
        return (
            dx,
            dw.to(w.dtype),
            db.to(w.dtype) if ctx.has_b else None,
            None,
            None,
        )


def fused_layer_norm(x, weight, bias=None, eps: float = 1e-5):
    if x.is_cuda:
        return _NormFn.apply(x, weight, bias, eps, False)
    return F.layer_norm(
        x.float(), (x.shape[-1],),
        weight.float(), bias.float() if bias is not None else None, eps
    ).to(x.dtype)


def fused_rms_norm(x, weight, eps: float = 1e-6):
    if x.is_cuda:
        return _NormFn.apply(x, weight, None, eps, True)
    xf = x.float()
    y = xf * torch.rsqrt(xf.pow(2).mean(-1, keepdim=True) + eps)
    return (y * weight.float()).to(x.dtype)


class FusedLayerNorm(torch.nn.Module):
    def __init__(self, dim: int, eps: float = 1e-5, bias: bool = True):
        super().__init__()
        self.eps = eps
        self.weight = torch.nn.Parameter(torch.ones(dim))
        self.bias = torch.nn.Parameter(torch.zeros(dim)) if bias else None

    def forward(self, x):
        return fused_layer_norm(x, self.weight, self.bias, self.eps)


class FusedRMSNorm(torch.nn.Module):
    def __init__(self, dim: int, eps: float = 1e-6):
        super().__init__()
        self.eps = eps
        self.weight = torch.nn.Parameter(torch.ones(dim))

    def forward(self, x):
        return fused_rms_norm(x, self.weight, self.eps)


class _CeFn(torch.autograd.Function):
    @staticmethod
    def forward(ctx, logits, targets_flat, Tr, ignore_index):
        ext = require_ext()
        loss, lse = ext.ce_fwd(logits, targets_flat, Tr, ignore_index)
        valid = (targets_flat != ignore_index).sum().clamp(min=1)
        ctx.save_for_backward(logits, targets_flat, lse, valid)
        ctx.Tr = Tr
        ctx.ignore_index = ignore_index
        return loss.sum() / valid.float()

    @staticmethod
    def backward(ctx, grad_out):
        ext = require_ext()
        logits, targets_flat, lse, valid = ctx.saved_tensors
        dloss = torch.full_like(lse, 0.0)
        dloss.fill_(1.0)
        dloss = dloss * (grad_out.float() / valid.float())
        dlogits = ext.ce_bwd(
            logits, targets_flat, lse, dloss, ctx.Tr, ctx.ignore_index
        )
        return dlogits, None, None, None


def fused_cross_entropy(
    logits: torch.Tensor,
    targets: torch.Tensor,
    shift: bool = True,
    ignore_index: int = -100,
) -> torch.Tensor:
    B, T, V = logits.shape
    if logits.is_cuda:
        Tr = T - 1 if shift else T
        tg = targets[:, 1:] if shift else targets
        return _CeFn.apply(
            logits.contiguous(), tg.contiguous().view(-1), Tr, ignore_index
        )
    if shift:
        lg = logits[:, :-1].float().reshape(-1, V)
        tg = targets[:, 1:].reshape(-1)
    else:
        lg = logits.float().reshape(-1, V)
        tg = targets.reshape(-1)
    return F.cross_entropy(lg, tg, ignore_index=ignore_index)


def rope_tables(
    T: int,
    rotary_dim: int,
    base: float = 10000.0,
    device=None,
    interleaved: bool = True,
) -> Tuple[torch.Tensor, torch.Tensor]:
    half = rotary_dim // 2
    inv = 1.0 / (base ** (torch.arange(0, half, dtype=torch.float32) * 2 / rotary_dim))
    t = torch.arange(T, dtype=torch.float32)
    freqs = torch.outer(t, inv)
    return freqs.cos().to(device), freqs.sin().to(device)


class _RopeFn(torch.autograd.Function):
    @staticmethod
    def forward(ctx, x, cos_t, sin_t, t_len, t_off, half_style):
        ext = require_ext()
        x = x.contiguous()
        y = torch.empty_like(x)
        ext.rope_apply(y, x, cos_t, sin_t, t_len, t_off, half_style, False)
        ctx.save_for_backward(cos_t, sin_t)
        ctx.meta = (t_len, t_off, half_style)
        return y

    @staticmethod
    def backward(ctx, dy):
        ext = require_ext()
        cos_t, sin_t = ctx.saved_tensors
        t_len, t_off, half_style = ctx.meta
        dy = dy.contiguous()
        dx = torch.empty_like(dy)
        ext.rope_apply(dx, dy, cos_t, sin_t, t_len, t_off, half_style, True)
        return dx, None, None, None, None, None


def _rope_cpu(x, cos_bt, sin_bt, half_style):
    B, T, H, D = x.shape
    half = cos_bt.shape[-1]
    c = cos_bt.view(B, T, 1, half).float()
    s = sin_bt.view(B, T, 1, half).float()
    xf = x.float()
    out = xf.clone()
    if half_style:
        x0 = xf[..., :half]
        x1 = xf[..., half : 2 * half]
        out[..., :half] = x0 * c - x1 * s
        out[..., half : 2 * half] = x1 * c + x0 * s
    else:
        x0 = xf[..., 0 : 2 * half : 2]
        x1 = xf[..., 1 : 2 * half : 2]
        out[..., 0 : 2 * half : 2] = x0 * c - x1 * s
        out[..., 1 : 2 * half : 2] = x1 * c + x0 * s
    return out.to(x.dtype)


def apply_rope(
    x: torch.Tensor,
    cos: torch.Tensor,
    sin: torch.Tensor,
    half_style: bool = False,
) -> torch.Tensor:
    B, T, H, D = x.shape
    half = cos.shape[-1]
    from saturn_amd.parallel.sequence import _STATE as _sp

    off = _sp["rank"] * T if _sp["world"] > 1 else 0
    if cos.shape[0] < off + T:
        raise ValueError(
            "rope table too short for this sequence shard — pass the FULL "
            "table to apply_rope (it slices positions itself)"
        )
    if cos.dtype != torch.float32:
        cos = cos.float()
        sin = sin.float()
    if x.is_cuda:
        return _RopeFn.apply(x, cos.contiguous(), sin.contiguous(), T, off,
                             half_style)
    cos_bt = cos[off : off + T].unsqueeze(0).expand(B, T, half)
    sin_bt = sin[off : off + T].unsqueeze(0).expand(B, T, half)
    return _rope_cpu(x, cos_bt.contiguous(), sin_bt.contiguous(), half_style)


def attention_math(q, k, v, causal: bool = True) -> torch.Tensor:
    scale = 1.0 / (q.shape[-1] ** 0.5)
    s = torch.matmul(q.float(), k.float().transpose(-1, -2)) * scale
    if causal:
        T = q.shape[-2]
        mask = torch.ones(T, T, dtype=torch.bool, device=q.device).tril()
        s = s.masked_fill(~mask, float("-inf"))
    p = torch.softmax(s, dim=-1)
    return torch.matmul(p, v.float()).to(q.dtype)


def _attention_core(q, k, v, causal: bool) -> torch.Tensor:
    if q.is_cuda:
        from saturn_amd.ops import flash

        return flash.flash_attention(q, k, v, causal=causal)
    if k.shape[1] != q.shape[1]:
        rep = q.shape[1] // k.shape[1]
        k = k.repeat_interleave(rep, dim=1)
        v = v.repeat_interleave(rep, dim=1)
    return attention_math(q, k, v, causal=causal)


def _attention(q, k, v, causal: bool) -> torch.Tensor:
    from saturn_amd.parallel.sequence import sp_attention, sp_world

    if sp_world() > 1:
        return sp_attention(q, k, v, lambda a, b, c: _attention_core(a, b, c, causal))
    return _attention_core(q, k, v, causal)


def causal_attention(q, k, v) -> torch.Tensor:
    return _attention(q, k, v, causal=True)


def full_attention(q, k, v) -> torch.Tensor:
    return _attention(q, k, v, causal=False)


class _Add3Fn(torch.autograd.Function):
    @staticmethod
    def forward(ctx, a, b, c):
        ext = require_ext()
        return ext.add3(a.contiguous(), b.contiguous(), c.contiguous())

    @staticmethod
    def backward(ctx, g):
        return g, g, g


def fused_add3(a, b, c):
    if a.is_cuda:
        return _Add3Fn.apply(a, b, c)
    return a + b + c


class _GeluFn(torch.autograd.Function):
    @staticmethod
    def forward(ctx, x):
        ext = require_ext()
        x = x.contiguous()
        ctx.save_for_backward(x)
        return ext.gelu_fwd(x)

    @staticmethod
    def backward(ctx, dy):
        ext = require_ext()
        (x,) = ctx.saved_tensors
        return ext.gelu_bwd(dy.contiguous(), x)


def fused_gelu(x: torch.Tensor) -> torch.Tensor:
    if x.is_cuda and x.dtype in (torch.bfloat16, torch.float16):
        return _GeluFn.apply(x)
    return torch.nn.functional.gelu(x, approximate="tanh")


_MLP_TN_DEFAULT = {"in": True, "out": True}


def _mlp_tn(site: str) -> bool:
    v = os.environ.get("SAMD_MLP_TN_" + site.upper())
    return _MLP_TN_DEFAULT[site] if v is None else v != "0"


def mlp_fused_supported(x, w_in, b_in, w_out, b_out) -> bool:
    if not (x.is_cuda and x.dtype == torch.bfloat16 and x.dim() >= 2):
        return False
    if b_in is None or b_out is None:
        return False
    if any(t.dtype != torch.bfloat16 or not t.is_cuda
           for t in (w_in, b_in, w_out, b_out)):
        return False
    E = x.shape[-1]
    M = x.numel() // E if E else 0
    F_ = w_in.shape[0]
    return (
        M > 0
        and w_in.shape == (F_, E)
        and w_out.shape == (E, F_)
        and M % 8 == 0
        and E % 8 == 0
        and F_ % 8 == 0
    )


class _GPTJMlpFn(torch.autograd.Function):

    @staticmethod
    def forward(ctx, h, w_in, b_in, w_out, b_out):
        ext = require_ext()
        pre = F.linear(h, w_in, b_in).contiguous()
        out = F.linear(ext.gelu_fwd(pre), w_out, b_out)
        ctx.save_for_backward(h, pre, w_in, w_out)
        return out

    @staticmethod
    def backward(ctx, g):
        ext = require_ext()
        h, pre, w_in, w_out = ctx.saved_tensors
        E = h.shape[-1]
        dh, dw_in, db_in, dw_out, db_out = ext.mlp_bwd(
            g.contiguous().view(-1, E),
            h.contiguous().view(-1, E),
            pre.view(-1, pre.shape[-1]),
            w_in.contiguous(),
            w_out.contiguous(),
            _mlp_tn("in"),
            _mlp_tn("out"),
        )
        return dh.view(h.shape), dw_in, db_in, dw_out, db_out


def gptj_mlp(h, w_in, b_in, w_out, b_out):
    return _GPTJMlpFn.apply(h, w_in, b_in, w_out, b_out)


_BLOCK_SITE_DEFAULT = {
    "SAMD_ATTN_TN_QKV": True,
    "SAMD_ATTN_TN_OUT": True,
    "SAMD_DH_ACCUM": False,
}


def _block_site(name: str) -> bool:
    v = os.environ.get(name)
    return _BLOCK_SITE_DEFAULT[name] if v is None else v != "0"


def _same_tensor(a, b) -> bool:
    return (
        a.data_ptr() == b.data_ptr()
        and a.shape == b.shape
        and a.stride() == b.stride()
    )


class _GPTJBranchesFn(torch.autograd.Function):

    @staticmethod
    def forward(ctx, h, wq, wk, wv, wo, w_in, b_in, w_out, b_out, cos, sin,
                n_head, t_off):
        ext = require_ext()
        B, T, E = h.shape
        D = E // n_head
        q = F.linear(h, wq).view(B, T, n_head, D)
        k = F.linear(h, wk).view(B, T, n_head, D)
        v = F.linear(h, wv).view(B, T, n_head, D)
        qr = torch.empty_like(q)
        ext.rope_apply(qr, q, cos, sin, T, t_off, False, False)
        kr = torch.empty_like(k)
        ext.rope_apply(kr, k, cos, sin, T, t_off, False, False)
        del q, k
        qr, kr, v = qr.transpose(1, 2), kr.transpose(1, 2), v.transpose(1, 2)
        o, lse = ext.attn_fwd(qr, kr, v, True, T)
        attn_out = F.linear(o.transpose(1, 2).reshape(B, T, E), wo)
        pre = F.linear(h, w_in, b_in).contiguous()
        mlp_out = F.linear(ext.gelu_fwd(pre), w_out, b_out)
        ctx.save_for_backward(h, pre, qr, kr, v, o, lse, wq, wk, wv, wo,
                              w_in, w_out, cos, sin)
        ctx.t_off = t_off
        return attn_out, mlp_out

    @staticmethod
    def backward(ctx, g_a, g_m):
        ext = require_ext()
        (h, pre, qr, kr, v, o, lse, wq, wk, wv, wo, w_in, w_out, cos,
         sin) = ctx.saved_tensors
        E = h.shape[-1]
        if g_a is None:
            g_a = torch.zeros_like(h)
        if g_m is None:
            g_m = torch.zeros_like(h)
        if _same_tensor(g_a, g_m):
            g_a = g_m = g_m.contiguous().view(-1, E)
        else:
            g_a = g_a.contiguous().view(-1, E)
            g_m = g_m.contiguous().view(-1, E)
        dh, dwq, dwk, dwv, dwo, dw_in, db_in, dw_out, db_out = (
            ext.gptj_branches_bwd(
                g_a, g_m,
                h.contiguous().view(-1, E),
                pre.view(-1, pre.shape[-1]),
                qr, kr, v, o, lse,
                wq.contiguous(), wk.contiguous(), wv.contiguous(),
                wo.contiguous(), w_in.contiguous(), w_out.contiguous(),
                cos, sin, ctx.t_off,
                _mlp_tn("in"), _mlp_tn("out"),
                _block_site("SAMD_ATTN_TN_QKV"),
                _block_site("SAMD_ATTN_TN_OUT"),
                _block_site("SAMD_DH_ACCUM"),
            )
        )
        return (dh.view(h.shape), dwq, dwk, dwv, dwo, dw_in, db_in, dw_out,
                db_out, None, None, None, None)


def gptj_branches_supported(h, n_head, rotary_dim, table_len) -> bool:
    if h.dim() != 3 or n_head <= 0:
        return False
    B, T, E = h.shape
    if E % n_head:
        return False
    D = E // n_head
    return (
        T % 64 == 0
        and T <= table_len
        and D in (64, 128, 256)
        and rotary_dim > 0
        and rotary_dim % 8 == 0
        and rotary_dim <= D
    )


def gptj_branches(h, wq, wk, wv, wo, w_in, b_in, w_out, b_out, cos, sin,
                  n_head):
    return _GPTJBranchesFn.apply(h, wq, wk, wv, wo, w_in, b_in, w_out, b_out,
                                 cos.contiguous(), sin.contiguous(), n_head, 0)


class _SwigluFn(torch.autograd.Function):
    @staticmethod
    def forward(ctx, gate, up):
        ext = require_ext()
        gate = gate.contiguous()
        up = up.contiguous()
        ctx.save_for_backward(gate, up)
        return ext.swiglu_fwd(gate, up)

    @staticmethod
    def backward(ctx, dout):
        ext = require_ext()
        gate, up = ctx.saved_tensors
        dgate, dup = ext.swiglu_bwd(dout.contiguous(), gate, up)
        return dgate, dup


def fused_swiglu(gate, up):
    if gate.is_cuda:
        return _SwigluFn.apply(gate, up)
    return torch.nn.functional.silu(gate) * up


class _EmbedFn(torch.autograd.Function):
    @staticmethod
    def forward(ctx, weight, idx):
        ext = require_ext()
        ctx.save_for_backward(idx)
        ctx.vocab = weight.shape[0]
        return ext.embed_fwd(weight, idx)

    @staticmethod
    def backward(ctx, dout):
        ext = require_ext()
        (idx,) = ctx.saved_tensors
        return ext.embed_bwd(dout, idx, ctx.vocab), None


def fused_embedding(weight, idx):
    if weight.is_cuda:
        return _EmbedFn.apply(weight, idx)
    return F.embedding(idx, weight)


class FusedEmbedding(torch.nn.Embedding):

    def forward(self, idx):
        if (
            self.weight.is_cuda
            and self.padding_idx is None
            and self.max_norm is None
            and not self.sparse
            and self.weight.dtype
            in (torch.bfloat16, torch.float16, torch.float32)
        ):
            return _EmbedFn.apply(self.weight, idx)
        return super().forward(idx)


class _DropoutFn(torch.autograd.Function):
    @staticmethod
    def forward(ctx, x, p, seed):
        ext = require_ext()
        ctx.p = p
        ctx.seed = seed
        return ext.dropout_fwd(x, p, seed)

    @staticmethod
    def backward(ctx, dout):
        ext = require_ext()
        return ext.dropout_bwd(dout.contiguous(), ctx.p, ctx.seed), None, None


def fused_dropout(x, p: float, training: bool = True):
    if p == 0.0 or not training:
        return x
    if x.is_cuda and x.dtype in (torch.bfloat16, torch.float16):
        seed = int(torch.randint(0, 2**62, (1,)).item())
        return _DropoutFn.apply(x.contiguous(), p, seed)
    return F.dropout(x, p, training)


class FusedDropout(torch.nn.Module):
    def __init__(self, p: float = 0.0):
        super().__init__()
        self.p = p

    def forward(self, x):
        return fused_dropout(x, self.p, self.training)

    def extra_repr(self):
        return f"p={self.p}"
```

Before: 63.43 samples/s.

## Fuse block layernorm into branch autograd and add attention-backward RoPE/transpose epilogue

Adds a fused autograd function that runs ln_1 together with the attention and MLP branches, so the layernorm backward can be folded into the branch backward kernel. The attention backward kernels gain an optional epilogue that un-rotates dQ/dK, writes the results in bf16 and also writes transposed copies, likely so the weight-gradient GEMMs can read them directly. A separate transpose-based LM-head backward is added but left disabled by default. The cost is more kernel template variants and extra LDS reuse, and correctness depends on the epilogue's RoPE inverse matching the forward rotation.

Result: faster. 64.12 samples/s (median of 6 runs) (+1.1%).

```diff
diff --git a/saturn_amd/models/gptj.py b/saturn_amd/models/gptj.py
--- a/saturn_amd/models/gptj.py
+++ b/saturn_amd/models/gptj.py
@@ -22,6 +22,9 @@
     mlp_fused_supported,
     gptj_branches,
     gptj_branches_supported,
+    gptj_branches_ln,
+    gptj_branches_ln_supported,
+    linear_head,
 )
 
 
@@ -158,6 +161,16 @@
         )
 
     def forward(self, x):
+        if gptj_branches_ln_supported(x, self.ln_1) and self._use_fused(x):
+            ln, attn, mlp = self.ln_1, self.attn, self.mlp
+            cos, sin = attn._rope(x.device)
+            a, m = gptj_branches_ln(
+                x, ln.weight, ln.bias, ln.eps,
+                attn.q_proj.weight, attn.k_proj.weight, attn.v_proj.weight,
+                attn.out_proj.weight, mlp.fc_in.weight, mlp.fc_in.bias,
+                mlp.fc_out.weight, mlp.fc_out.bias, cos, sin, attn.n_head,
+            )
+            return fused_add3(x, a, m)
         h = self.ln_1(x)
         if self._use_fused(h):
             attn, mlp = self.attn, self.mlp
@@ -196,7 +209,7 @@
         for block in self.h:
             x = block(x)
         x = self.ln_f(x)
-        return self.lm_head(x)
+        return linear_head(self.lm_head, x)
 
 
 def pretraining_loss(logits, labels):
@@ -219,7 +232,7 @@
         self.lm_head = lm_head
 
     def forward(self, x):
-        return self.lm_head(self.ln_f(x))
+        return linear_head(self.lm_head, self.ln_f(x))
 
 
 def as_sequential(model: GPTJForCausalLM) -> nn.Sequential:
diff --git a/saturn_amd/ops/csrc/attention.hip b/saturn_amd/ops/csrc/attention.hip
--- a/saturn_amd/ops/csrc/attention.hip
+++ b/saturn_amd/ops/csrc/attention.hip
@@ -590,7 +590,104 @@
   }
 }
 
-template <int D, bool TR16, bool VL2>
+struct AttnEpi {
+  const float* cos_t;
+  const float* sin_t;
+  unsigned short* t0;
+  unsigned short* t1;
+  long M;
+  long t_off;
+  int half;
+};
+
+template <bool ROT>
+__device__ __forceinline__ void attn_epi_vals(const f32x4& a, int dt, int r,
+                                              int tok0, const AttnEpi& ea,
+                                              unsigned short (&u)[4]) {
+  const int rot = 2 * ea.half;
+  const int col = dt * 16 + r;
+#pragma unroll
+  for (int reg = 0; reg < 4; ++reg) u[reg] = f2us(a[reg]);
+  if (ROT && dt * 16 < rot) {
+#pragma unroll
+    for (int reg = 0; reg < 4; ++reg) {
+      const float x = us2f(u[reg]);
+      const float xp = __shfl_xor(x, 1, 64);
+      if (col < rot) {
+        const long trow = (ea.t_off + tok0 + reg) * (long)ea.half;
+        const float c = ea.cos_t[trow + (col >> 1)];
+        const float s = -ea.sin_t[trow + (col >> 1)];
+        const float y = (r & 1) ? rope_rot_odd(xp, x, c, s)
+                                : rope_rot_even(x, xp, c, s);
+        u[reg] = fromF<c10::BFloat16>(y).x;
+      }
+    }
+  }
+}
+
+template <int D, bool ROT>
+__device__ __forceinline__ void attn_epi_store(const f32x4* acc, int tok0,
+                                               int r, unsigned short* rm,
+                                               long st, unsigned short* tr,
+                                               const AttnEpi& ea) {
+#pragma unroll
+  for (int dt = 0; dt < D / 16; ++dt) {
+    const int col = dt * 16 + r;
+    unsigned short u[4];
+    attn_epi_vals<ROT>(acc[dt], dt, r, tok0, ea, u);
+#pragma unroll
+    for (int reg = 0; reg < 4; ++reg) rm[(long)(tok0 + reg) * st + col] = u[reg];
+    uint2 pk;
+    pk.x = (unsigned)u[0] | ((unsigned)u[1] << 16);
+    pk.y = (unsigned)u[2] | ((unsigned)u[3] << 16);
+    *reinterpret_cast<uint2*>(tr + (long)col * ea.M + tok0) = pk;
+  }
+}
+
+template <int D>
+struct AttnEpiTile {
+  unsigned short rm[64][D + 8];
+  unsigned short tr[D][64 + 8];
+};
+
+template <int D, bool ROT>
+__device__ __forceinline__ void attn_epi_store_lds(
+    const f32x4* acc, AttnEpiTile<D>& tile, int tok_blk, int wid, int qg,
+    int r, unsigned short* rm, long st, unsigned short* tr,
+    const AttnEpi& ea) {
+  const int tl = wid * 16 + qg * 4;
+  __syncthreads();
+#pragma unroll
+  for (int dt = 0; dt < D / 16; ++dt) {
+    const int col = dt * 16 + r;
+    unsigned short u[4];
+    attn_epi_vals<ROT>(acc[dt], dt, r, tok_blk + tl, ea, u);
+#pragma unroll
+    for (int reg = 0; reg < 4; ++reg) tile.rm[tl + reg][col] = u[reg];
+    uint2 pk;
+    pk.x = (unsigned)u[0] | ((unsigned)u[1] << 16);
+    pk.y = (unsigned)u[2] | ((unsigned)u[3] << 16);
+    *reinterpret_cast<uint2*>(&tile.tr[col][tl]) = pk;
+  }
+  __syncthreads();
+  constexpr int VECS = (64 * D) / (256 * 8);
+#pragma unroll
+  for (int i = 0; i < VECS; ++i) {
+    const int idx = (i * 256 + threadIdx.x) * 8;
+    const int row = idx / D, col = idx % D;
+    *reinterpret_cast<bf16x8*>(rm + (long)(tok_blk + row) * st + col) =
+        *reinterpret_cast<const bf16x8*>(&tile.rm[row][col]);
+  }
+#pragma unroll
+  for (int i = 0; i < VECS; ++i) {
+    const int v = i * 256 + threadIdx.x;
+    const int col = v >> 3, mv = v & 7;
+    *reinterpret_cast<bf16x8*>(tr + (long)col * ea.M + tok_blk + mv * 8) =
+        *reinterpret_cast<const bf16x8*>(&tile.tr[col][mv * 8]);
+  }
+}
+
+template <int D, bool TR16, bool VL2, bool EPI>
 __launch_bounds__(256, 2)
 __global__ void attn_bwd_kernel(const unsigned short* __restrict__ dO,
                                 const unsigned short* __restrict__ Q,
@@ -605,7 +702,7 @@
                                 int n_kv, float scale, int causal,
                                 int kv_len, TStr dos,
                                 TStr qs, TStr ks, TStr vs,
-                                TStr dks, TStr dvs) {
+                                TStr dks, TStr dvs, AttnEpi ea) {
   using namespace bwd;
   extern __shared__ __attribute__((aligned(16))) char smem[];
   constexpr bool HASV = (D <= 128) && !VL2;
@@ -736,7 +833,18 @@
     __syncthreads();
   }
 
-  if (n_kv != n_heads) {
+  if constexpr (EPI) {
+    static_assert(sizeof(AttnEpiTile<D>) <= sizeof(AttnBwdLds<D, false>),
+                  "epilogue tile must fit the kernel's LDS");
+    AttnEpiTile<D>& tile = *reinterpret_cast<AttnEpiTile<D>*>(smem);
+    const long toff = h * (long)D * ea.M + b * (long)T;
+    attn_epi_store_lds<D, true>(acc_dk, tile, kv0, wid, qg, r,
+                                dK + b * dks.sb + h * dks.sh, dks.st,
+                                ea.t0 + toff, ea);
+    attn_epi_store_lds<D, false>(acc_dv, tile, kv0, wid, qg, r,
+                                 dV + b * dvs.sb + h * dvs.sh, dvs.st,
+                                 ea.t1 + toff, ea);
+  } else if (n_kv != n_heads) {
     float* dKh = dKf + b * dks.sb + h_kv * dks.sh;
     float* dVh = dVf + b * dvs.sb + h_kv * dvs.sh;
 #pragma unroll
@@ -780,7 +888,7 @@
   float delta_t[dq::QB];
 };
 
-template <int D, bool TR16, bool GKV>
+template <int D, bool TR16, bool GKV, bool EPI>
 __launch_bounds__(256, GKV ? 3 : (D <= 128 ? 2 : 1))
 __global__ void attn_dq_kernel(const unsigned short* __restrict__ dO,
                                const unsigned short* __restrict__ Q,
@@ -791,7 +899,7 @@
                                unsigned short* __restrict__ dQ16, int T,
                                int n_heads, int n_kv, float scale, int causal,
                                int kv_len, TStr dos, TStr qs, TStr ks,
-                               TStr vs, TStr dqs) {
+                               TStr vs, TStr dqs, AttnEpi ea) {
   using namespace dq;
   extern __shared__ __attribute__((aligned(16))) char smem[];
   AttnDqLds<D, GKV>& lds = *reinterpret_cast<AttnDqLds<D, GKV>*>(smem);
@@ -942,18 +1050,35 @@
   }
 
   unsigned short* dQh = dQ16 + b * dqs.sb + h * dqs.sh;
-#pragma unroll
-  for (int reg = 0; reg < 4; ++reg) {
-    const int q_glob = q0 + wid * 16 + qg * 4 + reg;
-#pragma unroll
-    for (int dt = 0; dt < D / 16; ++dt)
-      dQh[(long)q_glob * dqs.st + dt * 16 + r] = f2us(acc[dt][reg]);
-  }
-}
-
-std::vector<at::Tensor> attn_bwd(at::Tensor dout, at::Tensor q, at::Tensor k,
-                                 at::Tensor v, at::Tensor o, at::Tensor lse,
-                                 bool causal, int64_t kv_len) {
+  if constexpr (EPI) {
+    unsigned short* dQT = ea.t0 + h * (long)D * ea.M + b * (long)T;
+    if constexpr (GKV) {
+      attn_epi_store<D, true>(acc, q0 + wid * 16 + qg * 4, r, dQh, dqs.st,
+                              dQT, ea);
+    } else {
+      static_assert(sizeof(AttnEpiTile<D>) <= sizeof(AttnDqLds<D, false>),
+                    "epilogue tile must fit the kernel's LDS");
+      AttnEpiTile<D>& tile = *reinterpret_cast<AttnEpiTile<D>*>(smem);
+      attn_epi_store_lds<D, true>(acc, tile, q0, wid, qg, r, dQh, dqs.st, dQT,
+                                  ea);
+    }
+  } else {
+#pragma unroll
+    for (int reg = 0; reg < 4; ++reg) {
+      const int q_glob = q0 + wid * 16 + qg * 4 + reg;
+#pragma unroll
+      for (int dt = 0; dt < D / 16; ++dt)
+        dQh[(long)q_glob * dqs.st + dt * 16 + r] = f2us(acc[dt][reg]);
+    }
+  }
+}
+
+template <bool EPI>
+static std::vector<at::Tensor> attn_bwd_impl(at::Tensor dout, at::Tensor q,
+                                             at::Tensor k, at::Tensor v,
+                                             at::Tensor o, at::Tensor lse,
+                                             bool causal, int64_t kv_len,
+                                             AttnEpi eq, AttnEpi ekv) {
   using namespace bwd;
   TORCH_CHECK(q.is_cuda() && q.scalar_type() == at::kBFloat16);
   const int B = (int)q.size(0), H = (int)q.size(1), T = (int)q.size(2),
@@ -999,7 +1124,7 @@
     scale, causal ? 1 : 0, (int)kv_len, str_of(dout), str_of(q),             \
     str_of(k), str_of(v),                                                    \
     gqa ? str_of(dk_f32) : str_of(dk),                                       \
-    gqa ? str_of(dv_f32) : str_of(dv)
+    gqa ? str_of(dv_f32) : str_of(dv), ekv
 
 #define LAUNCH_B(DD)                                                         \
   do {                                                                       \
@@ -1016,11 +1141,11 @@
                        : sizeof(AttnDqLds<DD, false>);                       \
     static bool dq_attr_##DD = [] {                                          \
       hipFuncSetAttribute(                                                   \
-          reinterpret_cast<const void*>(&attn_dq_kernel<DD, false, false>),  \
+          reinterpret_cast<const void*>(&attn_dq_kernel<DD, false, false, EPI>),  \
           hipFuncAttributeMaxDynamicSharedMemorySize,                        \
           (int)sizeof(AttnDqLds<DD, false>));                                \
       hipFuncSetAttribute(                                                   \
-          reinterpret_cast<const void*>(&attn_dq_kernel<DD, true, false>),   \
+          reinterpret_cast<const void*>(&attn_dq_kernel<DD, true, false, EPI>),   \
           hipFuncAttributeMaxDynamicSharedMemorySize,                        \
           (int)sizeof(AttnDqLds<DD, false>));                                \
       return true;                                                           \
@@ -1029,7 +1154,7 @@
     {                                                                        \
       dim3 qgrid(B * H, T / dq::QB), qblock(256);                            \
       if (gkv)                                                               \
-        hipLaunchKernelGGL((attn_dq_kernel<DD, false, true>), qgrid,         \
+        hipLaunchKernelGGL((attn_dq_kernel<DD, false, true, EPI>), qgrid,         \
                            qblock, SH_DQ, stream.stream(),                   \
                            reinterpret_cast<const unsigned short*>(dout.data_ptr()), \
                            reinterpret_cast<const unsigned short*>(q.data_ptr()), \
@@ -1039,9 +1164,9 @@
                            reinterpret_cast<unsigned short*>(dq.data_ptr()), \
                            T, H, Hkv, scale, causal ? 1 : 0, (int)kv_len,   \
                            str_of(dout), str_of(q), str_of(k), str_of(v),    \
-                           str_of(dq));                                      \
+                           str_of(dq), eq);                                      \
       else if (bwd_is_tr16(DD))                                              \
-        hipLaunchKernelGGL((attn_dq_kernel<DD, true, false>), qgrid,         \
+        hipLaunchKernelGGL((attn_dq_kernel<DD, true, false, EPI>), qgrid,         \
                            qblock, SH_DQ, stream.stream(),                   \
                            reinterpret_cast<const unsigned short*>(dout.data_ptr()), \
                            reinterpret_cast<const unsigned short*>(q.data_ptr()), \
@@ -1051,9 +1176,9 @@
                            reinterpret_cast<unsigned short*>(dq.data_ptr()), \
                            T, H, Hkv, scale, causal ? 1 : 0, (int)kv_len,   \
                            str_of(dout), str_of(q), str_of(k), str_of(v),    \
-                           str_of(dq));                                      \
+                           str_of(dq), eq);                                      \
       else                                                                   \
-        hipLaunchKernelGGL((attn_dq_kernel<DD, false, false>), qgrid,        \
+        hipLaunchKernelGGL((attn_dq_kernel<DD, false, false, EPI>), qgrid,        \
                            qblock, SH_DQ, stream.stream(),                   \
                            reinterpret_cast<const unsigned short*>(dout.data_ptr()), \
                            reinterpret_cast<const unsigned short*>(q.data_ptr()), \
@@ -1063,7 +1188,7 @@
                            reinterpret_cast<unsigned short*>(dq.data_ptr()), \
                            T, H, Hkv, scale, causal ? 1 : 0, (int)kv_len,   \
                            str_of(dout), str_of(q), str_of(k), str_of(v),    \
-                           str_of(dq));                                      \
+                           str_of(dq), eq);                                      \
     }                                                                        \
     const bool tr = bwd_is_tr16(DD);                                         \
     const bool vl2 = bwd_is_vl2(DD);                                         \
@@ -1072,31 +1197,31 @@
     size_t shmem = vl2 ? SH_N : SH_V;                                        \
     static bool attr_set_##DD = [] {                                         \
       hipFuncSetAttribute(                                                   \
-          reinterpret_cast<const void*>(&attn_bwd_kernel<DD, false, false>), \
+          reinterpret_cast<const void*>(&attn_bwd_kernel<DD, false, false, EPI>), \
           hipFuncAttributeMaxDynamicSharedMemorySize, (int)SH_V);            \
       hipFuncSetAttribute(                                                   \
-          reinterpret_cast<const void*>(&attn_bwd_kernel<DD, true, false>),  \
+          reinterpret_cast<const void*>(&attn_bwd_kernel<DD, true, false, EPI>),  \
           hipFuncAttributeMaxDynamicSharedMemorySize, (int)SH_V);            \
       hipFuncSetAttribute(                                                   \
-          reinterpret_cast<const void*>(&attn_bwd_kernel<DD, false, true>),  \
+          reinterpret_cast<const void*>(&attn_bwd_kernel<DD, false, true, EPI>),  \
           hipFuncAttributeMaxDynamicSharedMemorySize, (int)SH_N);            \
       hipFuncSetAttribute(                                                   \
-          reinterpret_cast<const void*>(&attn_bwd_kernel<DD, true, true>),   \
+          reinterpret_cast<const void*>(&attn_bwd_kernel<DD, true, true, EPI>),   \
           hipFuncAttributeMaxDynamicSharedMemorySize, (int)SH_N);            \
       return true;                                                           \
     }();                                                                     \
     (void)attr_set_##DD;                                                     \
     if (tr && vl2)                                                           \
-      hipLaunchKernelGGL((attn_bwd_kernel<DD, true, true>), grid, block,     \
+      hipLaunchKernelGGL((attn_bwd_kernel<DD, true, true, EPI>), grid, block,     \
                          shmem, BWD_ARGS);                                   \
     else if (tr)                                                             \
-      hipLaunchKernelGGL((attn_bwd_kernel<DD, true, false>), grid, block,    \
+      hipLaunchKernelGGL((attn_bwd_kernel<DD, true, false, EPI>), grid, block,    \
                          shmem, BWD_ARGS);                                   \
     else if (vl2)                                                            \
-      hipLaunchKernelGGL((attn_bwd_kernel<DD, false, true>), grid, block,    \
+      hipLaunchKernelGGL((attn_bwd_kernel<DD, false, true, EPI>), grid, block,    \
                          shmem, BWD_ARGS);                                   \
     else                                                                     \
-      hipLaunchKernelGGL((attn_bwd_kernel<DD, false, false>), grid, block,   \
+      hipLaunchKernelGGL((attn_bwd_kernel<DD, false, false, EPI>), grid, block,   \
                          shmem, BWD_ARGS);                                   \
   } while (0)
 
@@ -1108,4 +1233,71 @@
   return {dq, dk, dv};
 }
 
-}
+std::vector<at::Tensor> attn_bwd(at::Tensor dout, at::Tensor q, at::Tensor k,
+                                 at::Tensor v, at::Tensor o, at::Tensor lse,
+                                 bool causal, int64_t kv_len) {
+  return attn_bwd_impl<false>(dout, q, k, v, o, lse, causal, kv_len,
+                              AttnEpi{}, AttnEpi{});
+}
+
+std::vector<at::Tensor> attn_bwd_rope_t(at::Tensor dout, at::Tensor q,
+                                        at::Tensor k, at::Tensor v,
+                                        at::Tensor o, at::Tensor lse,
+                                        at::Tensor cos_t, at::Tensor sin_t,
+                                        int64_t t_off, at::Tensor dqkvT) {
+  TORCH_CHECK(q.is_cuda() && q.scalar_type() == at::kBFloat16 && q.dim() == 4,
+              "attn_bwd_rope_t q: expected a bf16 GPU tensor [B, H, T, D]");
+  const long B = q.size(0), H = q.size(1), T = q.size(2), D = q.size(3);
+  TORCH_CHECK(k.dim() == 4 && k.size(1) == H,
+              "attn_bwd_rope_t: MHA only, got ", H, " q heads and ",
+              k.dim() == 4 ? k.size(1) : -1, " kv heads");
+  TORCH_CHECK(T > 0 && T % bwd::KB == 0,
+              "attn_bwd_rope_t: T must be a positive multiple of 64, got ", T);
+  TORCH_CHECK(D == 64 || D == 128 || D == 256,
+              "attn_bwd_rope_t: D in {64,128,256}");
+  for (const at::Tensor* t : {&dout, &k, &v, &o}) {
+    TORCH_CHECK(t->is_cuda() && t->device() == q.device() &&
+                    t->scalar_type() == at::kBFloat16 &&
+                    t->sizes() == q.sizes() && t->stride(3) == 1,
+                "attn_bwd_rope_t: dout, k, v, o must be bf16 [B, H, T, D] on "
+                "q's device with a dense last dim");
+  }
+  TORCH_CHECK(q.stride(3) == 1, "attn_bwd_rope_t: q needs a dense last dim");
+  TORCH_CHECK(lse.is_cuda() && lse.device() == q.device() &&
+                  lse.scalar_type() == at::kFloat && lse.is_contiguous() &&
+                  lse.dim() == 3 && lse.size(0) == B && lse.size(1) == H &&
+                  lse.size(2) == T,
+              "attn_bwd_rope_t lse: expected contiguous fp32 [B, H, T]");
+  for (const at::Tensor* t : {&cos_t, &sin_t}) {
+    TORCH_CHECK(t->is_cuda() && t->device() == q.device() &&
+                    t->scalar_type() == at::kFloat && t->dim() == 2 &&
+                    t->is_contiguous(),
+                "attn_bwd_rope_t: tables must be contiguous fp32 [T, half]");
+  }
+  TORCH_CHECK(sin_t.sizes() == cos_t.sizes(),
+              "attn_bwd_rope_t: table mismatch");
+  const long half = cos_t.size(1);
+  TORCH_CHECK(half > 0 && (2 * half) % 8 == 0 && 2 * half <= D,
+              "attn_bwd_rope_t: rotary dim ", 2 * half,
+              " must be a positive multiple of 8 within the head dim");
+  TORCH_CHECK(t_off >= 0 && cos_t.size(0) >= t_off + T,
+              "attn_bwd_rope_t: table too short for offset+T");
+  const long E = H * D, M = B * T;
+  TORCH_CHECK(dqkvT.is_cuda() && dqkvT.device() == q.device() &&
+                  dqkvT.scalar_type() == at::kBFloat16 && dqkvT.dim() == 2 &&
+                  dqkvT.is_contiguous() && dqkvT.size(0) == 3 * E &&
+                  dqkvT.size(1) == M,
+              "attn_bwd_rope_t: dqkvT must be contiguous bf16 [", 3 * E, ", ",
+              M, "]");
+  TORCH_CHECK(reinterpret_cast<uintptr_t>(dqkvT.data_ptr()) % 16 == 0,
+              "attn_bwd_rope_t: dqkvT must be 16-byte aligned");
+  auto* tbase = reinterpret_cast<unsigned short*>(dqkvT.data_ptr());
+  AttnEpi eq{cos_t.data_ptr<float>(), sin_t.data_ptr<float>(), tbase, nullptr,
+             M, (long)t_off, (int)half};
+  AttnEpi ekv = eq;
+  ekv.t0 = tbase + E * M;
+  ekv.t1 = tbase + 2 * E * M;
+  return attn_bwd_impl<true>(dout, q, k, v, o, lse, true, T, eq, ekv);
+}
+
+}
diff --git a/saturn_amd/ops/csrc/bindings.cpp b/saturn_amd/ops/csrc/bindings.cpp
--- a/saturn_amd/ops/csrc/bindings.cpp
+++ b/saturn_amd/ops/csrc/bindings.cpp
@@ -64,7 +64,26 @@
     at::Tensor k, at::Tensor v, at::Tensor o, at::Tensor lse, at::Tensor Wq,
     at::Tensor Wk, at::Tensor Wv, at::Tensor Wo, at::Tensor W_in,
     at::Tensor W_out, at::Tensor cos_t, at::Tensor sin_t, int64_t t_off,
-    bool tn_in, bool tn_out, bool tn_qkv, bool tn_o, bool dh_accum);
+    bool tn_in, bool tn_out, bool tn_qkv, bool tn_o, bool dh_accum,
+    bool attn_epi);
+std::vector<at::Tensor> norm_bwd_sum4(at::Tensor d0, at::Tensor d1,
+                                      at::Tensor d2, at::Tensor d3,
+                                      at::Tensor x, at::Tensor w,
+                                      at::Tensor mean, at::Tensor rstd,
+                                      bool needs_db);
+std::vector<at::Tensor> attn_bwd_rope_t(at::Tensor dout, at::Tensor q,
+                                        at::Tensor k, at::Tensor v,
+                                        at::Tensor o, at::Tensor lse,
+                                        at::Tensor cos_t, at::Tensor sin_t,
+                                        int64_t t_off, at::Tensor dqkvT);
+std::vector<at::Tensor> gptj_branches_ln_bwd(
+    at::Tensor g_a, at::Tensor g_m, at::Tensor x, at::Tensor ln_w,
+    at::Tensor mean, at::Tensor rstd, at::Tensor h, at::Tensor pre,
+    at::Tensor q, at::Tensor k, at::Tensor v, at::Tensor o, at::Tensor lse,
+    at::Tensor Wq, at::Tensor Wk, at::Tensor Wv, at::Tensor Wo,
+    at::Tensor W_in, at::Tensor W_out, at::Tensor cos_t, at::Tensor sin_t,
+    int64_t t_off, bool tn_in, bool tn_out, bool tn_qkv, bool tn_o,
+    bool dh_accum, bool attn_epi);
 }
 
 PYBIND11_MODULE(TORCH_EXTENSION_NAME, m) {
@@ -125,5 +144,27 @@
         py::arg("dy"), py::arg("cos"), py::arg("sin"), py::arg("t_len"),
         py::arg("t_off"), py::arg("dim"), py::arg("dxT"));
   m.def("gptj_branches_bwd", &samd::gptj_branches_bwd,
-        "GPT-J attention + MLP branch backward with shared transposes");
+        "GPT-J attention + MLP branch backward with shared transposes",
+        py::arg("g_a"), py::arg("g_m"), py::arg("h"), py::arg("pre"),
+        py::arg("q"), py::arg("k"), py::arg("v"), py::arg("o"),
+        py::arg("lse"), py::arg("Wq"), py::arg("Wk"), py::arg("Wv"),
+        py::arg("Wo"), py::arg("W_in"), py::arg("W_out"), py::arg("cos"),
+        py::arg("sin"), py::arg("t_off"), py::arg("tn_in"),
+        py::arg("tn_out"), py::arg("tn_qkv"), py::arg("tn_o"),
+        py::arg("dh_accum"), py::arg("attn_epi") = false);
+  m.def("norm_bwd_sum4", &samd::norm_bwd_sum4,
+        "LayerNorm backward of dy = ((d0 + d1) + d2) + d3, summed in-kernel "
+        "with add_'s roundings",
+        py::arg("d0"), py::arg("d1"), py::arg("d2"), py::arg("d3"),
+        py::arg("x"), py::arg("w"), py::arg("mean"), py::arg("rstd"),
+        py::arg("needs_db"));
+  m.def("attn_bwd_rope_t", &samd::attn_bwd_rope_t,
+        "causal MHA attention backward with the RoPE backward of dq/dk and "
+        "the stores of dq^T, dk^T, dv^T into a [3E, M] buffer in its epilogues",
+        py::arg("dout"), py::arg("q"), py::arg("k"), py::arg("v"),
+        py::arg("o"), py::arg("lse"), py::arg("cos"), py::arg("sin"),
+        py::arg("t_off"), py::arg("dqkvT"));
+  m.def("gptj_branches_ln_bwd", &samd::gptj_branches_ln_bwd,
+        "gptj_branches_bwd plus the backward of the LayerNorm that made h, "
+        "the dh sum folded into it");
 }
diff --git a/saturn_amd/ops/csrc/common.h b/saturn_amd/ops/csrc/common.h
--- a/saturn_amd/ops/csrc/common.h
+++ b/saturn_amd/ops/csrc/common.h
@@ -49,6 +49,15 @@
   unsigned int lsb = (c.i >> 16) & 1u;
   unsigned int rounded = c.i + 0x7fffu + lsb;
   return (unsigned short)(rounded >> 16);
+}
+
+__device__ __forceinline__ float rope_rot_even(float x0, float x1, float c,
+                                               float s) {
+  return __fmaf_rn(x0, c, -__fmul_rn(x1, s));
+}
+__device__ __forceinline__ float rope_rot_odd(float x0, float x1, float c,
+                                              float s) {
+  return __fmaf_rn(x1, c, __fmul_rn(x0, s));
 }
 
 __device__ __forceinline__ float wave_sum(float v) {
diff --git a/saturn_amd/ops/csrc/gptj_block_bwd.hip b/saturn_amd/ops/csrc/gptj_block_bwd.hip
--- a/saturn_amd/ops/csrc/gptj_block_bwd.hip
+++ b/saturn_amd/ops/csrc/gptj_block_bwd.hip
@@ -10,6 +10,19 @@
 std::vector<at::Tensor> attn_bwd(at::Tensor dout, at::Tensor q, at::Tensor k,
                                  at::Tensor v, at::Tensor o, at::Tensor lse,
                                  bool causal, int64_t kv_len);
+std::vector<at::Tensor> attn_bwd_rope_t(at::Tensor dout, at::Tensor q,
+                                        at::Tensor k, at::Tensor v,
+                                        at::Tensor o, at::Tensor lse,
+                                        at::Tensor cos_t, at::Tensor sin_t,
+                                        int64_t t_off, at::Tensor dqkvT);
+std::vector<at::Tensor> norm_bwd(at::Tensor dy, at::Tensor x, at::Tensor w,
+                                 at::Tensor mean, at::Tensor rstd, bool rms,
+                                 bool needs_db);
+std::vector<at::Tensor> norm_bwd_sum4(at::Tensor d0, at::Tensor d1,
+                                      at::Tensor d2, at::Tensor d3,
+                                      at::Tensor x, at::Tensor w,
+                                      at::Tensor mean, at::Tensor rstd,
+                                      bool needs_db);
 std::vector<at::Tensor> mlp_act_bwd(at::Tensor d_act, at::Tensor pre,
                                     bool want_dT, bool want_aT);
 void rope_apply(at::Tensor y, at::Tensor x, at::Tensor cos_t, at::Tensor sin_t,
@@ -61,8 +74,9 @@
           e1.x = (unsigned short)xv[2 * e + 1];
           const float x0 = toF<bf16_t>(e0);
           const float x1 = toF<bf16_t>(e1);
-          ov[i][2 * e] = (short)fromF<bf16_t>(x0 * c - x1 * s).x;
-          ov[i][2 * e + 1] = (short)fromF<bf16_t>(x1 * c + x0 * s).x;
+          ov[i][2 * e] = (short)fromF<bf16_t>(rope_rot_even(x0, x1, c, s)).x;
+          ov[i][2 * e + 1] =
+              (short)fromF<bf16_t>(rope_rot_odd(x0, x1, c, s)).x;
         }
       } else {
         ov[i] = xv;
@@ -142,12 +156,13 @@
   return dx;
 }
 
-std::vector<at::Tensor> gptj_branches_bwd(
+static std::vector<at::Tensor> branches_bwd_inner(
     at::Tensor g_a, at::Tensor g_m, at::Tensor h, at::Tensor pre, at::Tensor q,
     at::Tensor k, at::Tensor v, at::Tensor o, at::Tensor lse, at::Tensor Wq,
     at::Tensor Wk, at::Tensor Wv, at::Tensor Wo, at::Tensor W_in,
     at::Tensor W_out, at::Tensor cos_t, at::Tensor sin_t, int64_t t_off,
-    bool tn_in, bool tn_out, bool tn_qkv, bool tn_o, bool dh_accum) {
+    bool tn_in, bool tn_out, bool tn_qkv, bool tn_o, bool dh_accum,
+    bool attn_epi, std::vector<at::Tensor>* parts) {
   check_operand(g_a, "gptj_branches_bwd g_a");
   check_operand(g_m, "gptj_branches_bwd g_m");
   check_operand(h, "gptj_branches_bwd h");
@@ -212,10 +227,14 @@
     dWo = at::mm(g_a.t(), o2);
   }
 
-  at::Tensor dq_r, dk_r, dv;
+  const bool epi = attn_epi && tn_qkv;
+  at::Tensor dq_r, dk_r, dv, dqkvT;
+  if (tn_qkv) dqkvT = at::empty({3 * E, M}, h.options());
   {
-    auto r = attn_bwd(d_o.view({B, T, H, D}).permute({0, 2, 1, 3}), q, k, v, o,
-                      lse, true, T);
+    auto d_o4 = d_o.view({B, T, H, D}).permute({0, 2, 1, 3});
+    auto r = epi ? attn_bwd_rope_t(d_o4, q, k, v, o, lse, cos_t, sin_t, t_off,
+                                   dqkvT)
+                 : attn_bwd(d_o4, q, k, v, o, lse, true, T);
     dq_r = r[0].permute({0, 2, 1, 3});
     dk_r = r[1].permute({0, 2, 1, 3});
     dv = r[2].permute({0, 2, 1, 3});
@@ -228,12 +247,16 @@
 
   at::Tensor dq, dk, dWq, dWk, dWv;
   if (tn_qkv) {
-    auto dqkvT = at::empty({3 * E, M}, h.options());
-    dq = rope_bwd_t(dq_r, cos_t, sin_t, T, t_off, D, dqkvT.narrow(0, 0, E));
+    if (epi) {
+      dq = dq_r;
+      dk = dk_r;
+    } else {
+      dq = rope_bwd_t(dq_r, cos_t, sin_t, T, t_off, D, dqkvT.narrow(0, 0, E));
+      dk = rope_bwd_t(dk_r, cos_t, sin_t, T, t_off, D, dqkvT.narrow(0, E, E));
+      transpose_colsum_impl(dv2, false, true, dqkvT.narrow(0, 2 * E, E));
+    }
     dq_r.reset();
-    dk = rope_bwd_t(dk_r, cos_t, sin_t, T, t_off, D, dqkvT.narrow(0, E, E));
     dk_r.reset();
-    transpose_colsum_impl(dv2, false, true, dqkvT.narrow(0, 2 * E, E));
     auto dW = at::linear(dqkvT, hT);
     dqkvT.reset();
     hT.reset();
@@ -257,6 +280,9 @@
     dh.addmm_(dv2, Wv);
     dh.addmm_(dk2, Wk);
     dh.addmm_(dq2, Wq);
+  } else if (parts) {
+    *parts = {dh, at::mm(dv2, Wv), at::mm(dk2, Wk), at::mm(dq2, Wq)};
+    dh = at::Tensor();
   } else {
     dh.add_(at::mm(dv2, Wv));
     dh.add_(at::mm(dk2, Wk));
@@ -266,4 +292,42 @@
           dW_out, gt[1].to(W_out.scalar_type())};
 }
 
-}
+std::vector<at::Tensor> gptj_branches_bwd(
+    at::Tensor g_a, at::Tensor g_m, at::Tensor h, at::Tensor pre, at::Tensor q,
+    at::Tensor k, at::Tensor v, at::Tensor o, at::Tensor lse, at::Tensor Wq,
+    at::Tensor Wk, at::Tensor Wv, at::Tensor Wo, at::Tensor W_in,
+    at::Tensor W_out, at::Tensor cos_t, at::Tensor sin_t, int64_t t_off,
+    bool tn_in, bool tn_out, bool tn_qkv, bool tn_o, bool dh_accum,
+    bool attn_epi) {
+  return branches_bwd_inner(g_a, g_m, h, pre, q, k, v, o, lse, Wq, Wk, Wv, Wo,
+                            W_in, W_out, cos_t, sin_t, t_off, tn_in, tn_out,
+                            tn_qkv, tn_o, dh_accum, attn_epi, nullptr);
+}
+
+std::vector<at::Tensor> gptj_branches_ln_bwd(
+    at::Tensor g_a, at::Tensor g_m, at::Tensor x, at::Tensor ln_w,
+    at::Tensor mean, at::Tensor rstd, at::Tensor h, at::Tensor pre,
+    at::Tensor q, at::Tensor k, at::Tensor v, at::Tensor o, at::Tensor lse,
+    at::Tensor Wq, at::Tensor Wk, at::Tensor Wv, at::Tensor Wo,
+    at::Tensor W_in, at::Tensor W_out, at::Tensor cos_t, at::Tensor sin_t,
+    int64_t t_off, bool tn_in, bool tn_out, bool tn_qkv, bool tn_o,
+    bool dh_accum, bool attn_epi) {
+  check_operand(x, "gptj_branches_ln_bwd x");
+  TORCH_CHECK(x.sizes() == h.sizes() && x.device() == h.device(),
+              "gptj_branches_ln_bwd: x must match h");
+  TORCH_CHECK(x.size(1) <= 8192,
+              "gptj_branches_ln_bwd: row length above the vector LayerNorm "
+              "backward's 8192");
+  std::vector<at::Tensor> parts;
+  auto r = branches_bwd_inner(g_a, g_m, h, pre, q, k, v, o, lse, Wq, Wk, Wv,
+                              Wo, W_in, W_out, cos_t, sin_t, t_off, tn_in,
+                              tn_out, tn_qkv, tn_o, dh_accum, attn_epi,
+                              &parts);
+  auto n = dh_accum ? norm_bwd(r[0], x, ln_w, mean, rstd, false, true)
+                    : norm_bwd_sum4(parts[0], parts[1], parts[2], parts[3], x,
+                                    ln_w, mean, rstd, true);
+  return {n[0], n[1].to(ln_w.scalar_type()), n[2].to(ln_w.scalar_type()),
+          r[1], r[2], r[3], r[4], r[5], r[6], r[7], r[8]};
+}
+
+}
diff --git a/saturn_amd/ops/csrc/layernorm.hip b/saturn_amd/ops/csrc/layernorm.hip
--- a/saturn_amd/ops/csrc/layernorm.hip
+++ b/saturn_amd/ops/csrc/layernorm.hip
@@ -117,8 +117,33 @@
 }
 
 
-template <typename T, bool RMS, int GMAX>
+template <typename T, int NADD>
+__device__ __forceinline__ short8v_ln load_dy(const T* __restrict__ d0,
+                                              const T* __restrict__ d1,
+                                              const T* __restrict__ d2,
+                                              const T* __restrict__ d3,
+                                              long off) {
+  short8v_ln v = *reinterpret_cast<const short8v_ln*>(d0 + off);
+  if constexpr (NADD == 4) {
+    const short8v_ln v1 = *reinterpret_cast<const short8v_ln*>(d1 + off);
+    const short8v_ln v2 = *reinterpret_cast<const short8v_ln*>(d2 + off);
+    const short8v_ln v3 = *reinterpret_cast<const short8v_ln*>(d3 + off);
+#pragma unroll
+    for (int e = 0; e < 8; ++e) {
+      setElem<T>(v, e, elemF<T>(v, e) + elemF<T>(v1, e));
+      setElem<T>(v, e, elemF<T>(v, e) + elemF<T>(v2, e));
+      setElem<T>(v, e, elemF<T>(v, e) + elemF<T>(v3, e));
+    }
+  }
+  return v;
+}
+
+template <typename T, bool RMS, int GMAX, int NADD>
+__launch_bounds__(GMAX == 4 && NADD == 4 ? LN_BLOCK : 1024)
 __global__ void norm_bwd_vec_kernel(const T* __restrict__ dy,
+                                    const T* __restrict__ d1,
+                                    const T* __restrict__ d2,
+                                    const T* __restrict__ d3,
                                     const T* __restrict__ x,
                                     const T* __restrict__ w,
                                     const float* __restrict__ mean,
@@ -135,9 +160,9 @@
   float c_dyw[CACHE ? 8 * GMAX : 1];
   float c_xh[CACHE ? 8 * GMAX : 1];
   for (int row = blockIdx.x; row < rows; row += gridDim.x) {
-    const T* dyr = dy + (long)row * cols;
-    const T* xr = x + (long)row * cols;
-    T* dxr = dx + (long)row * cols;
+    const long roff = (long)row * cols;
+    const T* xr = x + roff;
+    T* dxr = dx + roff;
     const float mu = RMS ? 0.f : mean[row];
     const float rs = rstd[row];
     float s1 = 0.f, s2 = 0.f;
@@ -145,7 +170,7 @@
     for (int g = 0; g < GMAX; ++g) {
       const int j = (g * LN_BLOCK + threadIdx.x) * 8;
       if (j < cols) {
-        const short8v_ln dyv = *reinterpret_cast<const short8v_ln*>(dyr + j);
+        const short8v_ln dyv = load_dy<T, NADD>(dy, d1, d2, d3, roff + j);
         const short8v_ln xv = *reinterpret_cast<const short8v_ln*>(xr + j);
         const short8v_ln wv = *reinterpret_cast<const short8v_ln*>(w + j);
 #pragma unroll
@@ -177,7 +202,7 @@
             setElem<T>(ov, e,
                        rs * (c_dyw[g * 8 + e] - m1 - c_xh[g * 8 + e] * m2));
         } else {
-          const short8v_ln dyv = *reinterpret_cast<const short8v_ln*>(dyr + j);
+          const short8v_ln dyv = load_dy<T, NADD>(dy, d1, d2, d3, roff + j);
           const short8v_ln xv = *reinterpret_cast<const short8v_ln*>(xr + j);
           const short8v_ln wv = *reinterpret_cast<const short8v_ln*>(w + j);
 #pragma unroll
@@ -323,6 +348,46 @@
   return {y, mean, rstd};
 }
 
+template <typename T, int NADD>
+static void norm_bwd_vec_launch(const at::Tensor* const* d, const at::Tensor& x,
+                                const at::Tensor& w, const at::Tensor& mean,
+                                const at::Tensor& rstd, bool rms,
+                                bool needs_db, at::Tensor& dx, at::Tensor& dw,
+                                at::Tensor& db) {
+  const int cols = (int)x.size(-1);
+  const int rows = (int)(x.numel() / cols);
+  auto opts = x.options().dtype(at::kFloat);
+  auto stream = at::hip::getCurrentHIPStream();
+  dim3 grid(norm_grid(rows)), block(LN_BLOCK);
+  const int gneeded = (cols + 8 * LN_BLOCK - 1) / (8 * LN_BLOCK);
+  void (*kv)(const T*, const T*, const T*, const T*, const T*, const T*,
+             const float*, const float*, T*, float*, float*, int, int);
+  if (gneeded <= 2)
+    kv = rms ? norm_bwd_vec_kernel<T, true, 2, NADD>
+             : norm_bwd_vec_kernel<T, false, 2, NADD>;
+  else
+    kv = rms ? norm_bwd_vec_kernel<T, true, 4, NADD>
+             : norm_bwd_vec_kernel<T, false, 4, NADD>;
+  const int nblk = grid.x;
+  auto dw_part = at::empty({nblk, cols}, opts);
+  auto db_part = needs_db ? at::empty({nblk, cols}, opts) : at::Tensor();
+  auto ptr = [&](int i) {
+    return i < NADD ? reinterpret_cast<const T*>(d[i]->data_ptr()) : nullptr;
+  };
+  hipLaunchKernelGGL(kv, grid, block, 0, stream.stream(), ptr(0), ptr(1),
+                     ptr(2), ptr(3), reinterpret_cast<const T*>(x.data_ptr()),
+                     reinterpret_cast<const T*>(w.data_ptr()),
+                     rms ? nullptr : mean.data_ptr<float>(),
+                     rstd.data_ptr<float>(),
+                     reinterpret_cast<T*>(dx.data_ptr()),
+                     dw_part.data_ptr<float>(),
+                     needs_db ? db_part.data_ptr<float>() : nullptr, rows,
+                     cols);
+  SAMD_CHECK_HIP(hipGetLastError());
+  at::sum_out(dw, dw_part, {0});
+  if (needs_db) at::sum_out(db, db_part, {0});
+}
+
 std::vector<at::Tensor> norm_bwd(at::Tensor dy, at::Tensor x, at::Tensor w,
                                  at::Tensor mean, at::Tensor rstd, bool rms,
                                  bool needs_db) {
@@ -344,31 +409,9 @@
         using T = scalar_t;
         if constexpr (sizeof(T) == 2) {
           if (vec_ok) {
-            const int gneeded = (cols + 8 * LN_BLOCK - 1) / (8 * LN_BLOCK);
-            void (*kv)(const T*, const T*, const T*, const float*,
-                       const float*, T*, float*, float*, int, int);
-            if (gneeded <= 2)
-              kv = rms ? norm_bwd_vec_kernel<T, true, 2>
-                       : norm_bwd_vec_kernel<T, false, 2>;
-            else
-              kv = rms ? norm_bwd_vec_kernel<T, true, 4>
-                       : norm_bwd_vec_kernel<T, false, 4>;
-            const int nblk = grid.x;
-            auto dw_part = at::empty({nblk, cols}, opts);
-            auto db_part =
-                needs_db ? at::empty({nblk, cols}, opts) : at::Tensor();
-            hipLaunchKernelGGL(kv, grid, block, 0, stream.stream(),
-                               reinterpret_cast<const T*>(dy.data_ptr()),
-                               reinterpret_cast<const T*>(x.data_ptr()),
-                               reinterpret_cast<const T*>(w.data_ptr()),
-                               rms ? nullptr : mean.data_ptr<float>(),
-                               rstd.data_ptr<float>(),
-                               reinterpret_cast<T*>(dx.data_ptr()),
-                               dw_part.data_ptr<float>(),
-                               needs_db ? db_part.data_ptr<float>() : nullptr,
-                               rows, cols);
-            at::sum_out(dw, dw_part, {0});
-            if (needs_db) at::sum_out(db, db_part, {0});
+            const at::Tensor* d[1] = {&dy};
+            norm_bwd_vec_launch<T, 1>(d, x, w, mean, rstd, rms, needs_db, dx,
+                                      dw, db);
             return;
           }
         }
@@ -396,4 +439,56 @@
   return {dx, dw, db};
 }
 
-}
+std::vector<at::Tensor> norm_bwd_sum4(at::Tensor d0, at::Tensor d1,
+                                      at::Tensor d2, at::Tensor d3,
+                                      at::Tensor x, at::Tensor w,
+                                      at::Tensor mean, at::Tensor rstd,
+                                      bool needs_db) {
+  TORCH_CHECK(x.is_cuda() && x.is_contiguous() && x.dim() >= 1 &&
+                  x.numel() > 0,
+              "norm_bwd_sum4 x: expected a contiguous non-empty GPU tensor");
+  const long cols = x.size(-1);
+  const long rows = x.numel() / cols;
+  TORCH_CHECK(x.scalar_type() == at::kBFloat16 ||
+                  x.scalar_type() == at::kHalf,
+              "norm_bwd_sum4: expected a 16-bit floating type");
+  TORCH_CHECK(cols % 8 == 0 && cols <= 8 * LN_BLOCK * 4,
+              "norm_bwd_sum4: row length ", cols,
+              " must be a multiple of 8 and at most ", 8 * LN_BLOCK * 4);
+  const at::Tensor* d[4] = {&d0, &d1, &d2, &d3};
+  for (const at::Tensor* t : d) {
+    TORCH_CHECK(t->is_cuda() && t->device() == x.device() &&
+                    t->scalar_type() == x.scalar_type() &&
+                    t->is_contiguous() && t->numel() == x.numel() &&
+                    t->size(-1) == cols,
+                "norm_bwd_sum4: every addend must match x in device, type "
+                "and shape");
+    TORCH_CHECK(reinterpret_cast<uintptr_t>(t->data_ptr()) % 16 == 0,
+                "norm_bwd_sum4: addends must be 16-byte aligned");
+  }
+  TORCH_CHECK(reinterpret_cast<uintptr_t>(x.data_ptr()) % 16 == 0 &&
+                  reinterpret_cast<uintptr_t>(w.data_ptr()) % 16 == 0,
+              "norm_bwd_sum4: x and w must be 16-byte aligned");
+  TORCH_CHECK(w.is_cuda() && w.scalar_type() == x.scalar_type() &&
+                  w.is_contiguous() && w.numel() == cols,
+              "norm_bwd_sum4 w: expected [cols] of x's type");
+  auto f32_rows = [&](const at::Tensor& t) {
+    return t.is_cuda() && t.scalar_type() == at::kFloat &&
+           t.is_contiguous() && t.numel() == rows;
+  };
+  TORCH_CHECK(f32_rows(mean) && f32_rows(rstd),
+              "norm_bwd_sum4: mean and rstd must be fp32 [rows]");
+  auto dx = at::empty_like(x);
+  auto opts = x.options().dtype(at::kFloat);
+  auto dw = at::zeros({cols}, opts);
+  auto db = needs_db ? at::zeros({cols}, opts) : at::Tensor();
+  if (x.scalar_type() == at::kBFloat16)
+    norm_bwd_vec_launch<at::BFloat16, 4>(d, x, w, mean, rstd, false, needs_db,
+                                         dx, dw, db);
+  else
+    norm_bwd_vec_launch<at::Half, 4>(d, x, w, mean, rstd, false, needs_db, dx,
+                                     dw, db);
+  return {dx, dw, db};
+}
+
+}
diff --git a/saturn_amd/ops/functional.py b/saturn_amd/ops/functional.py
--- a/saturn_amd/ops/functional.py
+++ b/saturn_amd/ops/functional.py
@@ -347,6 +347,9 @@
     "SAMD_ATTN_TN_QKV": True,
     "SAMD_ATTN_TN_OUT": True,
     "SAMD_DH_ACCUM": False,
+    "SAMD_BLOCK_LN": True,
+    "SAMD_ATTN_EPI": True,
+    "SAMD_LMHEAD_TN": False,
 }
 
 
@@ -363,29 +366,60 @@
     )
 
 
+def _branches_forward(ext, h, wq, wk, wv, wo, w_in, b_in, w_out, b_out, cos,
+                      sin, n_head, t_off):
+    B, T, E = h.shape
+    D = E // n_head
+    q = F.linear(h, wq).view(B, T, n_head, D)
+    k = F.linear(h, wk).view(B, T, n_head, D)
+    v = F.linear(h, wv).view(B, T, n_head, D)
+    qr = torch.empty_like(q)
+    ext.rope_apply(qr, q, cos, sin, T, t_off, False, False)
+    kr = torch.empty_like(k)
+    ext.rope_apply(kr, k, cos, sin, T, t_off, False, False)
+    del q, k
+    qr, kr, v = qr.transpose(1, 2), kr.transpose(1, 2), v.transpose(1, 2)
+    o, lse = ext.attn_fwd(qr, kr, v, True, T)
+    attn_out = F.linear(o.transpose(1, 2).reshape(B, T, E), wo)
+    pre = F.linear(h, w_in, b_in).contiguous()
+    mlp_out = F.linear(ext.gelu_fwd(pre), w_out, b_out)
+    return attn_out, mlp_out, (h, pre, qr, kr, v, o, lse)
+
+
+def _branch_grads(g_a, g_m, h):
+    E = h.shape[-1]
+    if g_a is None:
+        g_a = torch.zeros_like(h)
+    if g_m is None:
+        g_m = torch.zeros_like(h)
+    if _same_tensor(g_a, g_m):
+        g_a = g_m = g_m.contiguous().view(-1, E)
+    else:
+        g_a = g_a.contiguous().view(-1, E)
+        g_m = g_m.contiguous().view(-1, E)
+    return g_a, g_m
+
+
+def _branch_sites():
+    return (
+        _mlp_tn("in"), _mlp_tn("out"),
+        _block_site("SAMD_ATTN_TN_QKV"),
+        _block_site("SAMD_ATTN_TN_OUT"),
+        _block_site("SAMD_DH_ACCUM"),
+        _block_site("SAMD_ATTN_EPI"),
+    )
+
+
 class _GPTJBranchesFn(torch.autograd.Function):
 
     @staticmethod
     def forward(ctx, h, wq, wk, wv, wo, w_in, b_in, w_out, b_out, cos, sin,
                 n_head, t_off):
         ext = require_ext()
-        B, T, E = h.shape
-        D = E // n_head
-        q = F.linear(h, wq).view(B, T, n_head, D)
-        k = F.linear(h, wk).view(B, T, n_head, D)
-        v = F.linear(h, wv).view(B, T, n_head, D)
-        qr = torch.empty_like(q)
-        ext.rope_apply(qr, q, cos, sin, T, t_off, False, False)
-        kr = torch.empty_like(k)
-        ext.rope_apply(kr, k, cos, sin, T, t_off, False, False)
-        del q, k
-        qr, kr, v = qr.transpose(1, 2), kr.transpose(1, 2), v.transpose(1, 2)
-        o, lse = ext.attn_fwd(qr, kr, v, True, T)
-        attn_out = F.linear(o.transpose(1, 2).reshape(B, T, E), wo)
-        pre = F.linear(h, w_in, b_in).contiguous()
-        mlp_out = F.linear(ext.gelu_fwd(pre), w_out, b_out)
-        ctx.save_for_backward(h, pre, qr, kr, v, o, lse, wq, wk, wv, wo,
-                              w_in, w_out, cos, sin)
+        attn_out, mlp_out, saved = _branches_forward(
+            ext, h, wq, wk, wv, wo, w_in, b_in, w_out, b_out, cos, sin,
+            n_head, t_off)
+        ctx.save_for_backward(*saved, wq, wk, wv, wo, w_in, w_out, cos, sin)
         ctx.t_off = t_off
         return attn_out, mlp_out
 
@@ -395,15 +429,7 @@
         (h, pre, qr, kr, v, o, lse, wq, wk, wv, wo, w_in, w_out, cos,
          sin) = ctx.saved_tensors
         E = h.shape[-1]
-        if g_a is None:
-            g_a = torch.zeros_like(h)
-        if g_m is None:
-            g_m = torch.zeros_like(h)
-        if _same_tensor(g_a, g_m):
-            g_a = g_m = g_m.contiguous().view(-1, E)
-        else:
-            g_a = g_a.contiguous().view(-1, E)
-            g_m = g_m.contiguous().view(-1, E)
+        g_a, g_m = _branch_grads(g_a, g_m, h)
         dh, dwq, dwk, dwv, dwo, dw_in, db_in, dw_out, db_out = (
             ext.gptj_branches_bwd(
                 g_a, g_m,
@@ -413,14 +439,66 @@
                 wq.contiguous(), wk.contiguous(), wv.contiguous(),
                 wo.contiguous(), w_in.contiguous(), w_out.contiguous(),
                 cos, sin, ctx.t_off,
-                _mlp_tn("in"), _mlp_tn("out"),
-                _block_site("SAMD_ATTN_TN_QKV"),
-                _block_site("SAMD_ATTN_TN_OUT"),
-                _block_site("SAMD_DH_ACCUM"),
+                *_branch_sites(),
             )
         )
         return (dh.view(h.shape), dwq, dwk, dwv, dwo, dw_in, db_in, dw_out,
                 db_out, None, None, None, None)
+
+
+class _GPTJBranchesFnLN(torch.autograd.Function):
+
+    @staticmethod
+    def forward(ctx, x, ln_w, ln_b, eps, wq, wk, wv, wo, w_in, b_in, w_out,
+                b_out, cos, sin, n_head, t_off):
+        ext = require_ext()
+        x = x.contiguous()
+        h, mean, rstd = ext.norm_fwd(x, ln_w, ln_b, eps, False)
+        attn_out, mlp_out, saved = _branches_forward(
+            ext, h, wq, wk, wv, wo, w_in, b_in, w_out, b_out, cos, sin,
+            n_head, t_off)
+        ctx.save_for_backward(x, ln_w, mean, rstd, *saved, wq, wk, wv, wo,
+                              w_in, w_out, cos, sin)
+        ctx.t_off = t_off
+        return attn_out, mlp_out
+
+    @staticmethod
+    def backward(ctx, g_a, g_m):
+        ext = require_ext()
+        (x, ln_w, mean, rstd, h, pre, qr, kr, v, o, lse, wq, wk, wv, wo,
+         w_in, w_out, cos, sin) = ctx.saved_tensors
+        E = h.shape[-1]
+        g_a, g_m = _branch_grads(g_a, g_m, h)
+        (dx, dln_w, dln_b, dwq, dwk, dwv, dwo, dw_in, db_in, dw_out,
+         db_out) = ext.gptj_branches_ln_bwd(
+            g_a, g_m,
+            x.view(-1, E), ln_w.contiguous(), mean, rstd,
+            h.view(-1, E),
+            pre.view(-1, pre.shape[-1]),
+            qr, kr, v, o, lse,
+            wq.contiguous(), wk.contiguous(), wv.contiguous(),
+            wo.contiguous(), w_in.contiguous(), w_out.contiguous(),
+            cos, sin, ctx.t_off,
+            *_branch_sites(),
+        )
+        return (dx.view(x.shape), dln_w, dln_b, None, dwq, dwk, dwv, dwo,
+                dw_in, db_in, dw_out, db_out, None, None, None, None)
+
+
+def gptj_branches_ln_supported(x, ln) -> bool:
+    if not _block_site("SAMD_BLOCK_LN"):
+        return False
+    if type(ln) is not FusedLayerNorm or ln.bias is None:
+        return False
+    if (ln._forward_hooks or ln._forward_pre_hooks or ln._backward_hooks
+            or ln._backward_pre_hooks):
+        return False
+    E = x.shape[-1]
+    if any(t.dtype != torch.bfloat16 or not t.is_cuda or t.shape != (E,)
+           for t in (ln.weight, ln.bias)):
+        return False
+    return (x.is_cuda and x.dtype == torch.bfloat16 and E % 8 == 0
+            and E <= 8192)
 
 
 def gptj_branches_supported(h, n_head, rotary_dim, table_len) -> bool:
@@ -444,6 +522,51 @@
                   n_head):
     return _GPTJBranchesFn.apply(h, wq, wk, wv, wo, w_in, b_in, w_out, b_out,
                                  cos.contiguous(), sin.contiguous(), n_head, 0)
+
+
+def gptj_branches_ln(x, ln_w, ln_b, eps, wq, wk, wv, wo, w_in, b_in, w_out,
+                     b_out, cos, sin, n_head):
+    return _GPTJBranchesFnLN.apply(x, ln_w, ln_b, eps, wq, wk, wv, wo, w_in,
+                                   b_in, w_out, b_out, cos.contiguous(),
+                                   sin.contiguous(), n_head, 0)
+
+
+class _LinearTNFn(torch.autograd.Function):
+    @staticmethod
+    def forward(ctx, x, w, b):
+        ctx.save_for_backward(x, w)
+        return F.linear(x, w, b)
+
+    @staticmethod
+    def backward(ctx, dy):
+        ext = require_ext()
+        x, w = ctx.saved_tensors
+        V, E = w.shape
+        dy2 = dy.contiguous().view(-1, V)
+        x2 = x.contiguous().view(-1, E)
+        dx = torch.mm(dy2, w).view(x.shape) if ctx.needs_input_grad[0] else None
+        dyT, db = ext.transpose_colsum(dy2, True)
+        xT, _ = ext.transpose_colsum(x2, False)
+        del dy2
+        return dx, F.linear(dyT, xT), db.to(w.dtype)
+
+
+def linear_head(head, x):
+    if (
+        _block_site("SAMD_LMHEAD_TN")
+        and type(head) is torch.nn.Linear
+        and head.bias is not None
+        and not (head._forward_hooks or head._forward_pre_hooks
+                 or head._backward_hooks or head._backward_pre_hooks)
+        and x.is_cuda and x.dtype == torch.bfloat16
+        and all(t.is_cuda and t.dtype == torch.bfloat16
+                for t in (head.weight, head.bias))
+        and x.shape[-1] == head.in_features
+        and head.in_features % 8 == 0 and head.out_features % 8 == 0
+        and x.numel() > 0 and (x.numel() // x.shape[-1]) % 8 == 0
+    ):
+        return _LinearTNFn.apply(x, head.weight, head.bias)
+    return head(x)
 
 
 class _SwigluFn(torch.autograd.Function):
```
